# chaoting-sun/GCT-Plus

Hardware: AMD Instinct MI355X
Metric: SMILES/sec training step (vaetf, seq_len=80, d_model=512) (higher is better)
Workload: dtype f32

## Files before the change

gct_plus_amd/csrc/attention.hip:

```cpp
#include "common.h"

typedef float f32x4 __attribute__((ext_vector_type(4)));

namespace {

constexpr int ATT_THREADS = 384;
constexpr int MASK_W = 8;
constexpr int L_MAX = 208;
constexpr int DIRECT_NT = GCT_ATTN_DIRECT_MAX_KEYS / 16;
constexpr int mask_words(int nt) { return (nt + 1) / 2; }
static_assert(GCT_ATTN_DIRECT_MAX_KEYS % 32 == 0 && mask_words(DIRECT_NT) == GCT_ATTN_DIRECT_MAX_KEYS / 32,
              "the direct kernels' rows are whole mask words");

struct AttnArgs {
  const float *q, *k, *v;
  int ldq, ldk, ldv;
  const uint32_t* mbits;
  int mb_sb, mb_sq;
  const uint32_t* tbits;
  int tb_sb, tb_su;
  float* o;
  int ldo;
  float* lse;
  float* probs;
  const float *o_in, *dout, *lse_in;
  float *dq, *dk, *dv;
  int lddq, lddk, lddv;
  const int32_t *cstart, *nlive;
  int kv_compact;
  int qo_compact;
  const int32_t *kstart, *klen;
  float4* ws_meta;
  uint32_t* ws_keep;
  uint32_t* ws_use;
  int B, H, Lq, Lk, npairs;
  float scale, keep_scale;
  uint32_t thr;
  GctRng rng;
#ifdef GCT_STAMPS
  unsigned long long* stamps;
#endif
};

#ifdef GCT_STAMPS
#define ASTAMP_DECL unsigned long long seg[8] = {0, 0, 0, 0, 0, 0, 0, 0}, tprev; \
  asm volatile("s_memtime %0\n\ts_waitcnt lgkmcnt(0)" : "=s"(tprev)::"memory")
#define ASTAMP(i)                                                                      \
  do {                                                                                 \
    __builtin_amdgcn_sched_barrier(0);                                                 \
    unsigned long long t__;                                                            \
    asm volatile("s_memtime %0\n\ts_waitcnt lgkmcnt(0)" : "=s"(t__)::"memory");         \
    __builtin_amdgcn_sched_barrier(0);                                                 \
    seg[i] += t__ - tprev;                                                             \
    tprev = t__;                                                                       \
  } while (0)
#define GCT_STAMP_ITEM0 8192
#define DSTAMP_OUT_AT(item, rec0)                                                      \
  if (a.stamps && (threadIdx.x & 63) == 0 && (item) >= GCT_STAMP_ITEM0 && (item) < GCT_STAMP_ITEM0 + 4096)  \
    for (int i = 0; i < 8; ++i) a.stamps[((size_t)((item) - GCT_STAMP_ITEM0 + (rec0))) * 8 + i] = seg[i]
#define DSTAMP_OUT(item) DSTAMP_OUT_AT(item, 0)
#else
#define ASTAMP_DECL
#define ASTAMP(i)
#define DSTAMP_OUT(item)
#define DSTAMP_OUT_AT(item, rec0)
#endif

__device__ __forceinline__ f32x4 mfma16(float a, float b, f32x4 c) {
  return __builtin_amdgcn_mfma_f32_16x16x4f32(a, b, c, 0, 0, 0);
}

template <int DK, int NT>
struct StageOff {
  static constexpr int C = DK / 4;
  static constexpr int ITERS = (16 * NT * C + ATT_THREADS - 1) / ATT_THREADS;
  uint32_t off[ITERS];
  __device__ __forceinline__ void init(int ld, int L, int tid) {
#pragma unroll
    for (int it = 0; it < ITERS; ++it) {
      const int idx = tid + it * ATT_THREADS;
      const int r = idx / C, c = idx - r * C;
      off[it] = (uint32_t)(((r < L ? r : L - 1) * ld + c * 4) * 4);
    }
  }
};
template <int DK, int NT>
struct Stage {
  static constexpr int SD = DK + 4, C = DK / 4;
  static constexpr int ITERS = StageOff<DK, NT>::ITERS;
  float4 v[ITERS];
  __device__ __forceinline__ void load(const float* src, int ld, int b, int h, int L, const StageOff<DK, NT>& o) {
    const float* base = src + (int64_t)b * L * ld + h * DK;
#pragma unroll
    for (int it = 0; it < ITERS; ++it)
      v[it] = *reinterpret_cast<const float4*>(reinterpret_cast<const char*>(base) + o.off[it]);
  }
  __device__ __forceinline__ void load_rows(const float* src, int ld, int64_t row0, int h, const StageOff<DK, NT>& o) {
    const float* base = src + row0 * ld + h * DK;
#pragma unroll
    for (int it = 0; it < ITERS; ++it)
      v[it] = *reinterpret_cast<const float4*>(reinterpret_cast<const char*>(base) + o.off[it]);
  }
  __device__ __forceinline__ void store(float* dst, int L, int LP, int tid) const {
#pragma unroll
    for (int it = 0; it < ITERS; ++it) {
      const int idx = tid + it * ATT_THREADS;
      const int r = idx / C, c = idx - r * C;
      if (r < LP)
        *reinterpret_cast<float4*>(dst + r * SD + c * 4) = r < L ? v[it] : make_float4(0.f, 0.f, 0.f, 0.f);
    }
  }
};

template <int NDT>
// ... 211 lines not shown
    sv.load_rows(a.v, a.ldv, kr0, h, kvo);
    row_frag_global<NDT>(bq, a.q, a.ldq, b, h, a.Lq, 16 * wave + c16, g);
    if (a.mbits) mask_row_raw<MW>(mraw, a, b, 16 * wave + c16);
  }
  for (;;) {
    const int b = pair / a.H, h = pair - b * a.H;
    const int Lk_in = a.klen ? a.klen[b] : a.Lk;
    sk.store(Ks, Lk_in, LKP, tid);
    sv.store(Vs, Lk_in, LKP, tid);
    uint32_t mw[MW];
    mask_row_use<MW>(mw, mraw, a, 16 * wave + c16);
    __syncthreads();
    const int next = pair + (int)gridDim.x;
    const bool more = next < a.npairs;
    const int nb = more ? next / a.H : b, nh = more ? next - nb * a.H : h;
    const int64_t nkr0 = a.kstart ? (int64_t)a.kstart[nb] : (int64_t)nb * a.Lk;
    if (PIPE && more) {
      sk.load_rows(a.k, a.ldk, nkr0, nh, kvo);
      sv.load_rows(a.v, a.ldv, nkr0, nh, kvo);
      if (a.mbits) mask_row_raw<MW>(mraw, a, nb, 16 * wave + c16);
    }
    for (int u = wave; u < nqt; u += NW) {
      if (u != wave) {
        row_frag_global<NDT>(bq, a.q, a.ldq, b, h, a.Lq, 16 * u + c16, g);
        uint4 r2[(MW + 3) / 4] = {};
        if (a.mbits) mask_row_raw<MW>(r2, a, b, 16 * u + c16);
        mask_row_use<MW>(mw, r2, a, 16 * u + c16);
      }
      const bool last = u + NW >= nqt;
      fwd_unit<NDT, NT, true>(a, b, h, u, bq, mw, Ks, Vs, nkt, lane, [&]() {
        if (PIPE && more && last) row_frag_global<NDT>(bq, a.q, a.ldq, nb, nh, a.Lq, 16 * wave + c16, g);
      });
    }
    if (PIPE && more && wave >= nqt) row_frag_global<NDT>(bq, a.q, a.ldq, nb, nh, a.Lq, 16 * wave + c16, g);
    if (!more) break;
    __syncthreads();
    if (!PIPE) {
      sk.load_rows(a.k, a.ldk, nkr0, nh, kvo);
      sv.load_rows(a.v, a.ldv, nkr0, nh, kvo);
      row_frag_global<NDT>(bq, a.q, a.ldq, nb, nh, a.Lq, 16 * wave + c16, g);
      if (a.mbits) mask_row_raw<MW>(mraw, a, nb, 16 * wave + c16);
    }
    pair = next;
  }
}

typedef float f32x2 __attribute__((ext_vector_type(2)));
template <int NDT> struct VecN;
template <> struct VecN<4> { typedef f32x4 T; };
template <> struct VecN<2> { typedef f32x2 T; };
template <> struct VecN<1> { typedef float T; };
template <int NDT> __device__ __forceinline__ float vec_at(const typename VecN<NDT>::T& v, int i);
template <> __device__ __forceinline__ float vec_at<4>(const f32x4& v, int i) { return v[i]; }
template <> __device__ __forceinline__ float vec_at<2>(const f32x2& v, int i) { return v[i]; }
template <> __device__ __forceinline__ float vec_at<1>(const float& v, int) { return v; }

template <int NDT>
struct WaveTile {
  static constexpr int SD = 16 * NDT + 4;
  typedef typename VecN<NDT>::T VT;
  float* t;
  __device__ __forceinline__ void put(const VT (&v)[4], int g, int c16) const {
#pragma unroll
    for (int r = 0; r < 4; ++r) *reinterpret_cast<VT*>(t + (4 * g + r) * SD + NDT * c16) = v[r];
  }
  __device__ __forceinline__ void get(float4 (&f)[NDT], int g, int c16) const {
    __builtin_amdgcn_wave_barrier();
#pragma unroll
    for (int j = 0; j < NDT; ++j) f[j] = *reinterpret_cast<const float4*>(t + c16 * SD + g * 4 * NDT + 4 * j);
    __builtin_amdgcn_wave_barrier();
  }
};
template <int NDT>
__device__ __forceinline__ void tile_load(typename VecN<NDT>::T (&v)[4], const char* base, int ld, int row0, int last,
                                          int g, int c16) {
  typedef typename VecN<NDT>::T VT;
#pragma unroll
  for (int r = 0; r < 4; ++r) {
    const int rr = row0 + 4 * g + r;
    v[r] = *reinterpret_cast<const VT*>(base + (uint32_t)(((rr < last ? rr : last) * ld + NDT * c16) * 4));
  }
}

template <int NDT, int NT>
__global__ __launch_bounds__(256, 6) void attn_fwd_direct_kernel(const AttnArgs a) {
  constexpr int DK = 16 * NDT, MW = mask_words(NT);
  typedef typename VecN<NDT>::T VT;
  const int lane = threadIdx.x & 63, g = lane >> 4, c16 = lane & 15;
  const int nqt = (a.Lq + 15) >> 4, nkt = (a.Lk + 15) >> 4;
  const int item = __builtin_amdgcn_readfirstlane((int)blockIdx.x * 4 + (int)(threadIdx.x >> 6));
  if (item >= a.npairs * nqt) return;
  ASTAMP_DECL;
  const int pair = item / nqt, u = item - pair * nqt;
  const int b = pair / a.H, h = pair - b * a.H;
  const int q = 16 * u + c16;
  const int Lq_e = a.qo_compact ? a.nlive[b] : a.Lq;
  const int64_t qr0 = a.qo_compact ? (int64_t)a.cstart[b] : (int64_t)b * a.Lq;
  if (16 * u >= Lq_e) return;
  const int Lk_in = a.klen ? a.klen[b] : a.Lk;
  const int64_t kr0 = a.kstart ? (int64_t)a.kstart[b] : (int64_t)b * a.Lk;
  const int klast = Lk_in > 0 ? Lk_in - 1 : 0;
  __shared__ __attribute__((aligned(16))) float tiles[4][16 * WaveTile<NDT>::SD];
  const int wv = threadIdx.x >> 6;
  const WaveTile<NDT> T0{tiles[wv]}, T1{tiles[wv]};
  VT tq[4];
  tile_load<NDT>(tq, reinterpret_cast<const char*>(a.q + qr0 * a.ldq + h * DK), a.ldq, 16 * u, Lq_e - 1, g, c16);
  uint4 mraw[(MW + 3) / 4] = {};
  if (a.mbits) mask_row_raw<MW>(mraw, a, b, q);
  const char* kbase = reinterpret_cast<const char*>(a.k + kr0 * a.ldk + h * DK);
  VT tk[4];
  uint32_t use = 0;
  if (a.tbits) {
    use = __builtin_amdgcn_readfirstlane(a.tbits[(int64_t)b * a.tb_sb + u * a.tb_su]);
    if (use & 1u) tile_load<NDT>(tk, kbase, a.ldk, 0, klast, g, c16);
  }
  uint32_t mw[MW];
  mask_row_use<MW>(mw, mraw, a, q);
  if (!a.tbits) {
    use = tiles_for_q<MW>(mw, q, a.Lq, a.Lk, nkt);
    if (use & 1u) tile_load<NDT>(tk, kbase, a.ldk, 0, klast, g, c16);
  }
  ASTAMP(0);
  uint32_t rowvis = 0;
#pragma unroll
  for (int w = 0; w < MW; ++w) rowvis |= mw[w] & range_word(w, a.Lk);
  float4 bq[NDT];
  T1.put(tq, g, c16);
  T1.get(bq, g, c16);
  ASTAMP(1);
  f32x4 sacc[NT];
#pragma unroll
  for (int t = 0; t < NT; ++t) sacc[t] = (f32x4){0.f, 0.f, 0.f, 0.f};
#pragma unroll
  for (int t = 0; t < NT; ++t) {
    if (t > 0 && ((use >> t) & 1u))
      tile_load<NDT>(tk, kbase, a.ldk, 16 * t, klast, g, c16);
    if ((use >> t) & 1u) {
      float4 ak[NDT];
      if (t & 1) {
        T1.put(tk, g, c16);
        T1.get(ak, g, c16);
      } else {
        T0.put(tk, g, c16);
        T0.get(ak, g, c16);
      }
      sacc[t] = dot_frag<NDT>(ak, bq, sacc[t]);
    }
  }
  ASTAMP(2);
  const char* vbase = reinterpret_cast<const char*>(a.v + kr0 * a.ldv + h * DK);
  VT av[4];
  if (use & 1u) tile_load<NDT>(av, vbase, a.ldv, 0, klast, g, c16);
  ASTAMP(3);
  float m = -INFINITY;
#pragma unroll
  for (int t = 0; t < NT; ++t)
    if ((use >> t) & 1u) {
      const uint32_t nib = mw[t >> 1] >> ((t & 1) * 16 + 4 * g);
#pragma unroll
      for (int r = 0; r < 4; ++r) {
        const float sv = score_of(sacc[t][r] * a.scale, 16 * t + 4 * g + r < a.Lk, (nib >> r) & 1u);
        sacc[t][r] = sv;
        m = fmaxf(m, sv);
      }
    }
  m = fmaxf(m, __shfl_xor(m, 16, 64));
  m = fmaxf(m, __shfl_xor(m, 32, 64));
  if (m == -INFINITY) m = 0.f;
  float l = 0.f;
#pragma unroll
  for (int t = 0; t < NT; ++t)
    if ((use >> t) & 1u) {
#pragma unroll
      for (int r = 0; r < 4; ++r) {
        const float e = __expf(sacc[t][r] - m);
        sacc[t][r] = e;
        l += e;
      }
    }
  l += __shfl_xor(l, 16, 64);
// ... 261 lines not shown
      const int kw = k >> 5, kb = k & 31;
      const bool inr = k < a.Lk;
#pragma unroll 1
      for (int u = 0; u < nqt; ++u) {
        if (!__any(rowlive[16 * u + c16] != 0)) continue;
        uint32_t vis4 = 0;
#pragma unroll
        for (int r = 0; r < 4; ++r) vis4 |= ((mb_s[(16 * u + 4 * g + r) * MW + kw] >> kb) & 1u) << r;
        const bool ok = __all(rowok[16 * u + c16] != 0);
        if (ok && !__any(inr && vis4 != 0)) continue;
        uint32_t keep4 = 0xfu;
        if (a.thr) {
          keep4 = 0;
#pragma unroll
          for (int r = 0; r < 4; ++r) keep4 |= ((kp_s[(16 * u + 4 * g + r) * MW + kw] >> kb) & 1u) << r;
        }
        f32x4 sa = (f32x4){0.f, 0.f, 0.f, 0.f}, pa = (f32x4){0.f, 0.f, 0.f, 0.f};
        {
          float4 aq[NDT], ad[NDT];
          row_frag<NDT>(aq, R0, 16 * u + c16, g);
          row_frag<NDT>(ad, R1, 16 * u + c16, g);
          sa = dot_frag<NDT>(aq, bk, sa);
          pa = dot_frag<NDT>(ad, bv, pa);
        }
        float pd[4], ds[4];
#pragma unroll
        for (int r = 0; r < 4; ++r) {
          const int qq = 16 * u + 4 * g + r;
          const bool vis = (vis4 >> r) & 1u, keep = (keep4 >> r) & 1u;
          const float p = inr ? __expf(score_of(sa[r] * a.scale, true, vis, rowok[qq] ? -1e9f : 0.f) - lse_s[qq]) : 0.f;
          const float dpd = keep ? pa[r] * a.keep_scale : 0.f;
          pd[r] = keep ? p * a.keep_scale : 0.f;
          ds[r] = (inr && vis) ? p * (dpd - del_s[qq]) : 0.f;
        }
#pragma unroll
        for (int r = 0; r < 4; ++r) {
          const float* dorow = R1 + (16 * u + 4 * g + r) * SD + c16;
          const float* qrow = R0 + (16 * u + 4 * g + r) * SD + c16;
#pragma unroll
          for (int dt = 0; dt < NDT; ++dt) {
            vacc[dt] = mfma16(dorow[16 * dt], pd[r], vacc[dt]);
            kacc[dt] = mfma16(qrow[16 * dt], ds[r], kacc[dt]);
          }
        }
      }
      if (k < Lk_e) {
        char* vbase = reinterpret_cast<char*>(a.dv + krow0 * a.lddv + h * DK);
        char* kbase = reinterpret_cast<char*>(a.dk + krow0 * a.lddk + h * DK);
        const uint32_t voff = (uint32_t)((k * a.lddv + 4 * g) * 4), koff = (uint32_t)((k * a.lddk + 4 * g) * 4);
#pragma unroll
        for (int dt = 0; dt < NDT; ++dt) {
          *reinterpret_cast<float4*>(vbase + voff + 64 * dt) = make_float4(vacc[dt][0], vacc[dt][1], vacc[dt][2], vacc[dt][3]);
          *reinterpret_cast<float4*>(kbase + koff + 64 * dt) =
              make_float4(kacc[dt][0] * a.scale, kacc[dt][1] * a.scale, kacc[dt][2] * a.scale, kacc[dt][3] * a.scale);
        }
      }
    }
    __syncthreads();
  }
}

template <int NDT>
struct DqBuf {
  typename VecN<NDT>::T kt[4], vt[4];
};

template <int NDT, int NT>
__global__ __launch_bounds__(256, 4) void attn_bwd_dq_kernel(const AttnArgs a) {
  constexpr int DK = 16 * NDT, MW = mask_words(NT);
  const int lane = threadIdx.x & 63, g = lane >> 4, c16 = lane & 15;
  const int nqt = (a.Lq + 15) >> 4, nkt = (a.Lk + 15) >> 4, LQP = 16 * nqt;
  const int item = __builtin_amdgcn_readfirstlane((int)blockIdx.x * 4 + (int)(threadIdx.x >> 6));
  if (item >= a.npairs * nqt) return;
  ASTAMP_DECL;
  const int pair = item / nqt, u = item - pair * nqt;
  const int b = pair / a.H, h = pair - b * a.H;
  const int64_t lrow0 = (int64_t)pair * a.Lq;
  const int Lq_e = a.nlive ? a.nlive[b] : a.Lq;
  const int64_t drow0 = a.cstart ? (int64_t)a.cstart[b] : (int64_t)b * a.Lq;
  const int64_t kin0 = a.kstart ? (int64_t)a.kstart[b] : (int64_t)b * a.Lk;
  const int Lk_in = a.klen ? a.klen[b] : a.Lk;
  const int klast = Lk_in > 0 ? Lk_in - 1 : 0;
  uint32_t* visit = a.ws_use + (int64_t)pair * nqt + u;
  if (16 * u >= Lq_e) {
    if (lane == 0) *visit = 0;
    return;
  }
  const int q = 16 * u + c16;
  const bool real = q < Lq_e;
  __shared__ __attribute__((aligned(16))) float tiles[4][2][16 * WaveTile<NDT>::SD];
  const int wv = threadIdx.x >> 6;
  const WaveTile<NDT> T0{tiles[wv][0]}, T1{tiles[wv][1]};
  DqBuf<NDT> b0;
  float4 bq[NDT], bd[NDT];
  float del = 0.f;
  int nz = 0;
  float lse0;
  uint4 mraw[(MW + 3) / 4] = {};
  {
    float4 bo[NDT];
    const int64_t qrow0 = a.qo_compact ? drow0 : (int64_t)b * a.Lq;
    const int qlast = (a.qo_compact ? Lq_e : a.Lq) - 1;
    const char* qb = reinterpret_cast<const char*>(a.q + qrow0 * a.ldq + h * DK);
    const char* db = reinterpret_cast<const char*>(a.dout + drow0 * a.ldo + h * DK);
    const char* ob = reinterpret_cast<const char*>(a.o_in + qrow0 * a.ldo + h * DK);
    tile_load<NDT>(b0.kt, qb, a.ldq, 16 * u, qlast, g, c16);
    tile_load<NDT>(b0.vt, db, a.ldo, 16 * u, Lq_e - 1, g, c16);
    lse0 = a.lse_in[lrow0 + (q < a.Lq ? q : a.Lq - 1)];
    if (a.mbits) mask_row_raw<MW>(mraw, a, b, q);
    T0.put(b0.kt, g, c16);
    T0.get(bq, g, c16);
    T1.put(b0.vt, g, c16);
    tile_load<NDT>(b0.kt, ob, a.ldo, 16 * u, qlast, g, c16);
    T1.get(bd, g, c16);
    T0.put(b0.kt, g, c16);
    T0.get(bo, g, c16);
#pragma unroll
    for (int j = 0; j < NDT; ++j) {
      del += (bo[j].x * bd[j].x + bo[j].y * bd[j].y) + (bo[j].z * bd[j].z + bo[j].w * bd[j].w);
      nz |= (bd[j].x != 0.f) | (bd[j].y != 0.f) | (bd[j].z != 0.f) | (bd[j].w != 0.f);
    }
  }
  ASTAMP(0);
  del += __shfl_xor(del, 16, 64);
  del += __shfl_xor(del, 32, 64);
  nz |= __shfl_xor(nz, 16, 64);
  nz |= __shfl_xor(nz, 32, 64);
  del = real ? del : 0.f;
  nz = real ? nz : 0;
  const float lse = real ? lse0 : 0.f;
  uint32_t mw[MW];
  mask_row_use<MW>(mw, mraw, a, q);
  uint32_t rowvis = 0;
#pragma unroll
  for (int w = 0; w < MW; ++w) rowvis |= mw[w] & range_word(w, a.Lk);
  const float masked = rowvis ? -1e9f : 0.f;
  if (g == 0) a.ws_meta[(int64_t)pair * LQP + q] = make_float4(lse, del, masked, nz ? 1.f : 0.f);
  const bool tile_live = __any(nz);
  char* dbase = reinterpret_cast<char*>(a.dq + drow0 * a.lddq + h * DK);
  const uint32_t doff = (uint32_t)((q * a.lddq + 4 * NDT * g) * 4);
  if (!tile_live) {
    if (lane == 0) *visit = 0;
    if (real) {
#pragma unroll
      for (int i = 0; i < NDT; ++i) *reinterpret_cast<float4*>(dbase + doff + 16 * i) = make_float4(0.f, 0.f, 0.f, 0.f);
    }
    return;
  }
  const uint32_t use = a.tbits ? __builtin_amdgcn_readfirstlane(a.tbits[(int64_t)b * a.tb_sb + u * a.tb_su])
                               : tiles_for_q<MW>(mw, q, a.Lq, a.Lk, nkt);
  if (lane == 0) *visit = use;
  const uint64_t keepw = keep_bits_row<NT>(a, (uint32_t)(lrow0 + q), use, g);
  ASTAMP(1);
  uint16_t* kp_h = reinterpret_cast<uint16_t*>(a.ws_keep + ((int64_t)pair * LQP + q) * MW);
  const char* kbase = reinterpret_cast<const char*>(a.k + kin0 * a.ldk + h * DK);
  const char* vbase = reinterpret_cast<const char*>(a.v + kin0 * a.ldv + h * DK);
  auto load = [&](DqBuf<NDT>& B_, int t) {
    tile_load<NDT>(B_.kt, kbase, a.ldk, 16 * t, klast, g, c16);
    tile_load<NDT>(B_.vt, vbase, a.ldv, 16 * t, klast, g, c16);
  };
  f32x4 qacc[NDT];
#pragma unroll
  for (int dt = 0; dt < NDT; ++dt) qacc[dt] = (f32x4){0.f, 0.f, 0.f, 0.f};
  auto compute = [&](const DqBuf<NDT>& B_, int t) {
    ASTAMP(2);
    f32x4 sacc = (f32x4){0.f, 0.f, 0.f, 0.f}, pacc = (f32x4){0.f, 0.f, 0.f, 0.f};
    {
      float4 ak[NDT];
      T0.put(B_.kt, g, c16);
      T0.get(ak, g, c16);
      sacc = dot_frag<NDT>(ak, bq, sacc);
      T1.put(B_.vt, g, c16);
      T1.get(ak, g, c16);
      pacc = dot_frag<NDT>(ak, bd, pacc);
    }
    ASTAMP(3);
    uint32_t word = mw[0];
#pragma unroll
    for (int w = 1; w < MW; ++w) word = (t >> 1) == w ? mw[w] : word;
    const uint32_t nib = word >> ((t & 1) * 16 + 4 * g);
    const uint32_t keep = (uint32_t)(keepw >> (4 * t)) & 0xfu;
    if (a.thr) {
      uint32_t hw = keep << (4 * g);
      hw |= __shfl_xor(hw, 16, 64);
      hw |= __shfl_xor(hw, 32, 64);
      if (g == 0) kp_h[t] = (uint16_t)hw;
    }
    float ds[4];
#pragma unroll
    for (int r = 0; r < 4; ++r) {
      const bool inr = 16 * t + 4 * g + r < a.Lk, vis = (nib >> r) & 1u;
      const float p = inr ? __expf(score_of(sacc[r] * a.scale, true, vis, masked) - lse) : 0.f;
      const float dpd = ((keep >> r) & 1u) ? pacc[r] * a.keep_scale : 0.f;
      ds[r] = (inr && vis) ? p * (dpd - del) : 0.f;
    }
    ASTAMP(4);
#pragma unroll
    for (int r = 0; r < 4; ++r) {
#pragma unroll
      for (int dt = 0; dt < NDT; ++dt) qacc[dt] = mfma16(vec_at<NDT>(B_.kt[r], dt), ds[r], qacc[dt]);
    }
    ASTAMP(5);
  };
  for (uint32_t rem = use; rem; rem &= rem - 1) {
    const int t0 = __builtin_ctz(rem);
    load(b0, t0);
    compute(b0, t0);
  }
  if (real) {
#pragma unroll
    for (int i = 0; i < 4; ++i) {
      if constexpr (NDT == 4)
        *reinterpret_cast<float4*>(dbase + doff + 16 * i) =
            make_float4(qacc[0][i] * a.scale, qacc[1][i] * a.scale, qacc[2][i] * a.scale, qacc[3][i] * a.scale);
      else if constexpr (NDT == 2)
        *reinterpret_cast<float2*>(dbase + doff + 8 * i) = make_float2(qacc[0][i] * a.scale, qacc[1][i] * a.scale);
      else
        *reinterpret_cast<float*>(dbase + doff + 4 * i) = qacc[0][i] * a.scale;
    }
  }
  ASTAMP(6);
  DSTAMP_OUT_AT(item, 4096);
}

template <int NDT>
struct DkvBuf {
  typename VecN<NDT>::T tq[4], td[4];
};

template <int NDT, int NT>
__global__ __launch_bounds__(256, 4) void attn_bwd_dkv_kernel(const AttnArgs a) {
  constexpr int DK = 16 * NDT, MW = mask_words(NT);
  const int lane = threadIdx.x & 63, g = lane >> 4, c16 = lane & 15;
  const int nqt = (a.Lq + 15) >> 4, nkt = (a.Lk + 15) >> 4, LQP = 16 * nqt;
  const int item = __builtin_amdgcn_readfirstlane((int)blockIdx.x * 4 + (int)(threadIdx.x >> 6));
  if (item >= a.npairs * nkt) return;
  ASTAMP_DECL;
  const int pair = item / nkt, t = item - pair * nkt;
  const int b = pair / a.H, h = pair - b * a.H;
  const int Lq_e = a.nlive ? a.nlive[b] : a.Lq;
  const int64_t drow0 = a.cstart ? (int64_t)a.cstart[b] : (int64_t)b * a.Lq;
  const int64_t kin0 = a.kstart ? (int64_t)a.kstart[b] : (int64_t)b * a.Lk;
  const int Lk_in = a.klen ? a.klen[b] : a.Lk;
  const int Lk_e = a.kv_compact ? Lq_e : Lk_in;
  const int64_t krow0 = a.kv_compact ? drow0 : kin0;
  if (16 * t >= Lk_e) return;
  const int k = 16 * t + c16;
  const bool inr = k < a.Lk;
  uint32_t rem = 0;
  {
    const uint32_t* vw = a.ws_use + (int64_t)pair * nqt;
    const int Lq_x = Lq_e < a.Lq ? Lq_e : a.Lq;
    const int nqt_e = (Lq_x + 15) >> 4;
    for (int u = 0; u < nqt_e; ++u) rem |= ((vw[u] >> t) & 1u) << u;
    rem = __builtin_amdgcn_readfirstlane(rem);
  }
  __shared__ __attribute__((aligned(16))) float tiles[4][2][16 * WaveTile<NDT>::SD];
  const int wv = threadIdx.x >> 6;
  const WaveTile<NDT> T0{tiles[wv][0]}, T1{tiles[wv][1]};
  float4 bk[NDT], bv[NDT];
  DkvBuf<NDT> b0;
  {
    DkvBuf<NDT>& kv = b0;
    const char* kb0 = reinterpret_cast<const char*>(a.k + kin0 * a.ldk + h * DK);
    const char* vb0 = reinterpret_cast<const char*>(a.v + kin0 * a.ldv + h * DK);
    const int klast = Lk_in > 0 ? Lk_in - 1 : 0;
    tile_load<NDT>(kv.tq, kb0, a.ldk, 16 * t, klast, g, c16);
    tile_load<NDT>(kv.td, vb0, a.ldv, 16 * t, klast, g, c16);
    T0.put(kv.tq, g, c16);
    T1.put(kv.td, g, c16);
    T0.get(bk, g, c16);
    T1.get(bv, g, c16);
  }
  ASTAMP(0);
  f32x4 vacc[NDT], kacc[NDT];
#pragma unroll
  for (int dt = 0; dt < NDT; ++dt) {
    vacc[dt] = (f32x4){0.f, 0.f, 0.f, 0.f};
    kacc[dt] = (f32x4){0.f, 0.f, 0.f, 0.f};
  }
  const int kw = t >> 1, kb = (t & 1) * 16 + c16;
  const float4* meta = a.ws_meta + (int64_t)pair * LQP;
  const uint32_t* kp = a.ws_keep + (int64_t)pair * LQP * MW + kw;
  const uint32_t* mb = a.mbits ? a.mbits + (int64_t)b * a.mb_sb + kw : nullptr;
  const int64_t qrow0 = a.qo_compact ? drow0 : (int64_t)b * a.Lq;
  const int qlast = (a.qo_compact ? Lq_e : a.Lq) - 1;
  const char* qbase = reinterpret_cast<const char*>(a.q + qrow0 * a.ldq + h * DK);
  const char* dbase = reinterpret_cast<const char*>(a.dout + drow0 * a.ldo + h * DK);
  auto load = [&](DkvBuf<NDT>& B_, int u) {
    tile_load<NDT>(B_.tq, qbase, a.ldq, 16 * u, qlast, g, c16);
    tile_load<NDT>(B_.td, dbase, a.ldo, 16 * u, Lq_e - 1, g, c16);
  };
  auto compute = [&](const DkvBuf<NDT>& B_, int u) {
    float4 mt[4];
    uint32_t mword[4], kword[4];
    {
      const int qq = 16 * u + 4 * g + (c16 & 3);
      const int qc = qq < a.Lq ? qq : a.Lq - 1;
      const float4 m1 = meta[qq];
      const uint32_t w1 = mb ? mb[qc * a.mb_sq] : 0xffffffffu;
      const uint32_t k1 = a.thr ? kp[qq * MW] : 0xffffffffu;
#define GCT_QUAD(v, r) __builtin_amdgcn_mov_dpp((int)(v), (r) * 0x55, 0xf, 0xf, true)
#pragma unroll
      for (int r = 0; r < 4; ++r) {
        mt[r].x = __int_as_float(r == 0 ? GCT_QUAD(__float_as_int(m1.x), 0) : r == 1 ? GCT_QUAD(__float_as_int(m1.x), 1)
                               : r == 2 ? GCT_QUAD(__float_as_int(m1.x), 2) : GCT_QUAD(__float_as_int(m1.x), 3));
        mt[r].y = __int_as_float(r == 0 ? GCT_QUAD(__float_as_int(m1.y), 0) : r == 1 ? GCT_QUAD(__float_as_int(m1.y), 1)
                               : r == 2 ? GCT_QUAD(__float_as_int(m1.y), 2) : GCT_QUAD(__float_as_int(m1.y), 3));
        mt[r].z = __int_as_float(r == 0 ? GCT_QUAD(__float_as_int(m1.z), 0) : r == 1 ? GCT_QUAD(__float_as_int(m1.z), 1)
                               : r == 2 ? GCT_QUAD(__float_as_int(m1.z), 2) : GCT_QUAD(__float_as_int(m1.z), 3));
        mt[r].w = 0.f;
        mword[r] = (uint32_t)(r == 0 ? GCT_QUAD(w1, 0) : r == 1 ? GCT_QUAD(w1, 1) : r == 2 ? GCT_QUAD(w1, 2) : GCT_QUAD(w1, 3));
        kword[r] = (uint32_t)(r == 0 ? GCT_QUAD(k1, 0) : r == 1 ? GCT_QUAD(k1, 1) : r == 2 ? GCT_QUAD(k1, 2) : GCT_QUAD(k1, 3));
      }
#undef GCT_QUAD
    }
    ASTAMP(1);
    f32x4 sa = (f32x4){0.f, 0.f, 0.f, 0.f}, pa = (f32x4){0.f, 0.f, 0.f, 0.f};
    {
      float4 aq[NDT];
      T0.put(B_.tq, g, c16);
      T1.put(B_.td, g, c16);
      T0.get(aq, g, c16);
      sa = dot_frag<NDT>(aq, bk, sa);
      T1.get(aq, g, c16);
      pa = dot_frag<NDT>(aq, bv, pa);
    }
    ASTAMP(2);
// ... 193 lines not shown
  const int per_cu = lds <= 50 * 1024 ? 3 : lds <= 76 * 1024 ? 2 : 1;
  const int64_t want = (int64_t)cus * per_cu * 2;
  return {nt8 ? AttnRoute::LDS8 : AttnRoute::LDS13, npairs < want ? npairs : want, 0, lds};
}

struct BwdWs {
  int64_t keep, use, bytes;
};
BwdWs bwd_ws_layout(int B, int H, int Lq) {
  const int64_t LQP = (Lq + 15) & ~15, rows = (int64_t)B * H * LQP;
  const int64_t keep = rows * 16, use = keep + rows * mask_words(DIRECT_NT) * 4;
  return {keep, use, use + (((int64_t)B * H * (LQP / 16) * 4 + 15) & ~(int64_t)15)};
}

template <typename K>
int launch_lds(K kernel, const AttnRoute& r, const AttnArgs& a, hipStream_t st) {
  int rc = ensure_lds(kernel, r.lds);
  if (rc) return rc;
  hipLaunchKernelGGL(kernel, dim3((unsigned)r.grid), dim3(ATT_THREADS), r.lds, st, a);
  return GCT_OK;
}

template <bool BWD, int NDT>
int launch_route(const AttnRoute& r, const AttnArgs& a, hipStream_t st) {
  switch (r.kind) {
    case AttnRoute::DIRECT:
      if constexpr (BWD) {
        hipLaunchKernelGGL((attn_bwd_dq_kernel<NDT, DIRECT_NT>), dim3((unsigned)r.grid), dim3(256), 0, st, a);
        hipLaunchKernelGGL((attn_bwd_dkv_kernel<NDT, DIRECT_NT>), dim3((unsigned)r.grid_kv), dim3(256), 0, st, a);
      } else {
        hipLaunchKernelGGL((attn_fwd_direct_kernel<NDT, DIRECT_NT>), dim3((unsigned)r.grid), dim3(256), 0, st, a);
      }
      return GCT_OK;
    case AttnRoute::LDS8:
      return BWD ? launch_lds(attn_bwd_kernel<NDT, 8>, r, a, st) : launch_lds(attn_fwd_kernel<NDT, 8>, r, a, st);
    default:
      return BWD ? launch_lds(attn_bwd_kernel<NDT, 13>, r, a, st) : launch_lds(attn_fwd_kernel<NDT, 13>, r, a, st);
  }
}

template <bool BWD>
int launch(int dk, const AttnRoute& r, const AttnArgs& a, hipStream_t st) {
  switch (dk) {
    case 64: return launch_route<BWD, 4>(r, a, st);
    case 32: return launch_route<BWD, 2>(r, a, st);
    default: return launch_route<BWD, 1>(r, a, st);
  }
}

}

extern "C" int gct_attn_mask_pack(const uint8_t* mask, int64_t mask_sb, int64_t mask_sq, int B, int Lq, int Lk,
                                  uint32_t* bits, uint32_t* tiles, void* stream) {
  GCT_CHECK_ARG(mask && bits && B >= 0 && Lq > 0 && Lk > 0 && Lk <= 32 * MASK_W && gct_aligned16(bits),
                "attn_mask_pack: bad args (Lk <= %d)", 32 * MASK_W);
  const int rows = mask_sq == 0 ? 1 : Lq;
  const int64_t n = (int64_t)B * rows * MASK_W;
  if (n == 0) return GCT_OK;
  hipLaunchKernelGGL(mask_pack_kernel, dim3((unsigned)((n + 255) / 256)), dim3(256), 0, (hipStream_t)stream, mask,
                     mask_sb, mask_sq, B, rows, Lk, bits);
  GCT_LAUNCH_CHECK("attn_mask_pack");
  if (tiles) {
    const int ntr = mask_sq == 0 ? 1 : (Lq + 15) / 16;
    const int64_t items = (int64_t)B * ntr;
    hipLaunchKernelGGL(mask_tiles_kernel, dim3((unsigned)((items + 3) / 4)), dim3(256), 0, (hipStream_t)stream, bits,
                       rows * MASK_W, mask_sq == 0 ? 0 : MASK_W, B, ntr, Lq, Lk, tiles);
    GCT_LAUNCH_CHECK("attn_mask_pack (tiles)");
  }
  return GCT_OK;
}

extern "C" int gct_trg_mask_tokens(const int64_t* tokens, int64_t ld_tok, int64_t pad, int B, int T, uint8_t* out,
                                   void* stream) {
  GCT_CHECK_ARG(tokens && out && B >= 0 && T > 0 && ld_tok >= T && ((uintptr_t)out & 3u) == 0,
                "trg_mask_tokens: bad args");
  const int64_t n4 = ((int64_t)B * T * T + 3) / 4;
  if (n4 == 0) return GCT_OK;
  hipLaunchKernelGGL(trg_mask_tokens_kernel, dim3((unsigned)((n4 + 255) / 256)), dim3(256), 0, (hipStream_t)stream,
                     tokens, ld_tok, pad, B, T, out);
  GCT_LAUNCH_CHECK("trg_mask_tokens");
  return GCT_OK;
}

extern "C" int gct_attn_fwd(const float* q, int64_t ldq, const float* k, int64_t ldk,
                            const float* v, int64_t ldv, const uint32_t* mbits, int64_t mb_sb,
                            int64_t mb_sq, float* o, int64_t ldo, float* lse, float* probs, int B,
                            int H, int Lq, int Lk, int dk, float scale, float p, uint64_t seed,
                            uint32_t site, const int32_t* kstart, const int32_t* klen, const uint32_t* tbits,
                            int64_t tb_sb, int64_t tb_su, const int32_t* qstart, const int32_t* qlen, void* stream) {
  int rc = check_common("attn_fwd", q, ldq, k, ldk, v, ldv, mbits, mb_sb, mb_sq, B, H, Lq, Lk, dk, p);
  if (rc) return rc;
  GCT_CHECK_ARG(o && lse && ldo % 4 == 0 && gct_aligned16(o) && (int64_t)Lq * ldo * 4 < (1ll << 31), "attn_fwd: bad output");
  if (B == 0) return GCT_OK;
  AttnArgs a = {};
  a.q = q; a.k = k; a.v = v; a.ldq = (int)ldq; a.ldk = (int)ldk; a.ldv = (int)ldv;
  a.mbits = mbits; a.mb_sb = (int)mb_sb; a.mb_sq = (int)mb_sq;
  a.o = o; a.ldo = (int)ldo; a.lse = lse; a.probs = probs;
  a.tbits = tbits; a.tb_sb = (int)tb_sb; a.tb_su = (int)tb_su;
#ifdef GCT_STAMPS
  a.stamps = g_attn_stamps;
#endif
  GCT_CHECK_ARG((kstart == nullptr) == (klen == nullptr), "attn_fwd: kstart / klen go together");
  a.kstart = kstart; a.klen = klen;
  GCT_CHECK_ARG((qstart == nullptr) == (qlen == nullptr), "attn_fwd: qstart / qlen go together");
  GCT_CHECK_ARG(!qstart || (Lk <= GCT_ATTN_DIRECT_MAX_KEYS && !probs),
                "attn_fwd: compact query rows need the direct kernel (Lk <= %d) and no probs output",
                GCT_ATTN_DIRECT_MAX_KEYS);
  a.cstart = qstart; a.nlive = qlen; a.qo_compact = qstart ? 1 : 0;
  a.B = B; a.H = H; a.Lq = Lq; a.Lk = Lk; a.npairs = B * H; a.scale = scale;
  a.thr = gct_drop_threshold(p); a.keep_scale = 1.0f / (1.0f - p); a.rng = gct_rng_make(seed, site);
  rc = launch<false>(dk, plan_attn_fwd(Lq, Lk, dk, a.npairs, num_cus()), a, (hipStream_t)stream);
  if (rc) return rc;
  GCT_LAUNCH_CHECK("attn_fwd");
  return GCT_OK;
}

extern "C" int64_t gct_attn_bwd_ws_bytes(int B, int H, int Lq, int Lk) {
  if (B <= 0 || H <= 0 || Lq <= 0 || Lk <= 0 || Lk > GCT_ATTN_DIRECT_MAX_KEYS) return 0;
  return bwd_ws_layout(B, H, Lq).bytes;
}

extern "C" int gct_attn_bwd(const float* q, int64_t ldq, const float* k, int64_t ldk,
                            const float* v, int64_t ldv, const uint32_t* mbits, int64_t mb_sb,
                            int64_t mb_sq, const float* o, const float* dout, int64_t ldo,
                            const float* lse, float* dq, int64_t lddq, float* dk_,
                            int64_t lddk, float* dv, int64_t lddv, int B, int H, int Lq, int Lk,
                            int dk, float scale, float p, uint64_t seed, uint32_t site,
                            const int32_t* cstart, const int32_t* nlive, int kv_compact,
                            const int32_t* kstart, const int32_t* klen, const uint32_t* tbits, int64_t tb_sb,
                            int64_t tb_su, void* ws, int64_t ws_bytes, void* stream) {
  int rc = check_common("attn_bwd", q, ldq, k, ldk, v, ldv, mbits, mb_sb, mb_sq, B, H, Lq, Lk, dk, p);
  if (rc) return rc;
  GCT_CHECK_ARG(o && dout && lse && dq && dk_ && dv, "attn_bwd: null pointer");
  GCT_CHECK_ARG(ldo % 4 == 0 && lddq % 4 == 0 && lddk % 4 == 0 && lddv % 4 == 0 &&
                    gct_aligned16(o) && gct_aligned16(dout) && gct_aligned16(dq) &&
                    gct_aligned16(dk_) && gct_aligned16(dv),
                "attn_bwd: buffers must be 16-B aligned with ld %% 4 == 0");
  GCT_CHECK_ARG((int64_t)Lq * (ldo > lddq ? ldo : lddq) * 4 < (1ll << 31) && (int64_t)Lk * (lddk > lddv ? lddk : lddv) * 4 < (1ll << 31),
                "attn_bwd: one (batch) slice exceeds 2 GiB");
  if (B == 0) return GCT_OK;
  AttnArgs a = {};
  a.q = q; a.k = k; a.v = v; a.ldq = (int)ldq; a.ldk = (int)ldk; a.ldv = (int)ldv;
  a.mbits = mbits; a.mb_sb = (int)mb_sb; a.mb_sq = (int)mb_sq;
  a.o_in = o; a.dout = dout; a.ldo = (int)ldo; a.lse_in = lse;
  a.tbits = tbits; a.tb_sb = (int)tb_sb; a.tb_su = (int)tb_su;
  a.dq = dq; a.dk = dk_; a.dv = dv; a.lddq = (int)lddq; a.lddk = (int)lddk; a.lddv = (int)lddv;
#ifdef GCT_STAMPS
  a.stamps = g_attn_stamps;
#endif
  const int qo_compact = (kv_compact >> 1) & 1;
  kv_compact &= 1;
  GCT_CHECK_ARG((cstart == nullptr) == (nlive == nullptr) && (!kv_compact || (cstart && Lq == Lk)),
                "attn_bwd: cstart / nlive go together; kv_compact needs them and Lq == Lk");
  GCT_CHECK_ARG(!qo_compact || cstart, "attn_bwd: compact q / o rows need cstart / nlive");
  a.cstart = cstart; a.nlive = nlive; a.kv_compact = kv_compact; a.qo_compact = qo_compact;
  GCT_CHECK_ARG((kstart == nullptr) == (klen == nullptr) && !(kstart && kv_compact),
                "attn_bwd: kstart / klen go together and exclude kv_compact");
  a.kstart = kstart; a.klen = klen;
  GCT_CHECK_ARG(!qo_compact || Lk <= GCT_ATTN_DIRECT_MAX_KEYS,
                "attn_bwd: compact q / o rows need the direct kernels (Lk <= %d)", GCT_ATTN_DIRECT_MAX_KEYS);
  const int64_t ws_need = gct_attn_bwd_ws_bytes(B, H, Lq, Lk);
  GCT_CHECK_ARG(ws_need == 0 || (ws && gct_aligned16(ws) && ws_bytes >= ws_need),
                "attn_bwd: Lk <= %d needs a 16-B aligned workspace of %lld B (gct_attn_bwd_ws_bytes); got %lld B at %p",
                GCT_ATTN_DIRECT_MAX_KEYS, (long long)ws_need, (long long)ws_bytes, ws);
  a.B = B; a.H = H; a.Lq = Lq; a.Lk = Lk; a.npairs = B * H; a.scale = scale;
  a.thr = gct_drop_threshold(p); a.keep_scale = 1.0f / (1.0f - p); a.rng = gct_rng_make(seed, site);
  const AttnRoute r = plan_attn_bwd(Lq, Lk, dk, a.npairs, num_cus());
  GCT_CHECK_ARG(r.grid <= INT32_MAX && r.grid_kv <= INT32_MAX, "attn_bwd: grid too large");
  if (r.kind == AttnRoute::DIRECT) {
    const BwdWs w = bwd_ws_layout(B, H, Lq);
    a.ws_meta = reinterpret_cast<float4*>(ws);
    a.ws_keep = reinterpret_cast<uint32_t*>(static_cast<char*>(ws) + w.keep);
    a.ws_use = reinterpret_cast<uint32_t*>(static_cast<char*>(ws) + w.use);
  }
  rc = launch<true>(dk, r, a, (hipStream_t)stream);
  if (rc) return rc;
  GCT_LAUNCH_CHECK("attn_bwd");
  return GCT_OK;
}
```

gct_plus_amd/csrc/gemm.hip:

```cpp
#include <limits.h>
#include <stdlib.h>

#include "common.h"

typedef float f32x16 __attribute__((ext_vector_type(16)));

namespace {

constexpr int BM = 128, BN = 128, BK = 32;
constexpr int TILE_FLOATS = BM * BK;

struct Seg3 {
  const float* p0;
  int64_t d1, d2;
};

struct GemmArgs {
  int64_t M, N, K;
  Seg3 a;
  int64_t lda;
  int64_t a_nper;
  Seg3 b;
  int64_t ldb;
  int64_t b_nper;
// ... 240 lines not shown
#ifdef GCT_STAMPS
  unsigned long long seg[8] = {0, 0, 0, 0, 0, 0, 0, 0}, tprev;
  asm volatile("s_memtime %0\n\ts_waitcnt lgkmcnt(0)" : "=s"(tprev)::"memory");
#endif
  if (nkt > 0) {
    gload(kbeg);
    lstore(0);
  }
  __syncthreads();
  STAMP(0);
  for (int64_t kt = 0; kt < nkt; ++kt) {
    const int cur = (int)(kt & 1);
    if (kt + 1 < nkt) gload(kbeg + (kt + 1) * BK);
    STAMP(1);
    const float* la = lds + cur * 2 * TILE_FLOATS;
    const float* lb = la + TILE_FLOATS;
    float fa[2][2][4], fb[2][2][4];
    auto fragq = [&](int set, int c) {
      if (A_KC) fragq_kc(fa[set], la, wm, lane, c); else fragq_rc(fa[set], la, wm, lane, c);
      if (B_KC) fragq_kc(fb[set], lb, wn, lane, c); else fragq_rc(fb[set], lb, wn, lane, c);
    };
    fragq(0, 0);
#pragma unroll
    for (int c = 0; c < 4; ++c) {
      const int set = c & 1;
      if (c < 3) fragq(set ^ 1, c + 1);
      __builtin_amdgcn_sched_barrier(0);
#pragma unroll
      for (int e = 0; e < 4; ++e) {
#pragma unroll
        for (int i = 0; i < 2; ++i)
#pragma unroll
          for (int j = 0; j < 2; ++j)
            acc[i][j] = __builtin_amdgcn_mfma_f32_32x32x2f32(fa[set][i][e], fb[set][j][e], acc[i][j],
                                                             0, 0, 0);
      }
      __builtin_amdgcn_sched_barrier(0);
    }
    STAMP(2);
#ifdef GCT_STAMPS
    asm volatile("s_waitcnt vmcnt(0)" ::: "memory");
    STAMP(3);
#endif
    if (kt + 1 < nkt) lstore(cur ^ 1);
    STAMP(4);
    __syncthreads();
    STAMP(5);
  }

  const int h = lane >> 5;
#pragma unroll
  for (int i = 0; i < 2; ++i) {
#pragma unroll
    for (int j = 0; j < 2; ++j) {
      const int64_t col = n0 + wn + j * 32 + (lane & 31);
      if (col >= g.N) continue;
      int64_t cloc;
      float* cbase;
      float bias = 0.f;
      if (g.epi == EPI_SLAB) {
        cbase = g.c0 + (int64_t)z * g.slab_stride;
        cloc = col;
      } else {
        const bool g1 = col >= g.c_nper, g2 = col >= 2 * g.c_nper;
        cloc = col - (g2 ? 2 * g.c_nper : (g1 ? g.c_nper : 0));
        cbase = g.c0 + (g2 ? g.c_d2 : (g1 ? g.c_d1 : 0));
        if (g.epi < EPI_D0 && g.bias0)
          bias = g.bias0[(g2 ? g.bias_d2 : (g1 ? g.bias_d1 : 0)) + cloc];
      }
#pragma unroll
      for (int q4 = 0; q4 < 4; ++q4) {
        const int64_t row_base = m0 + wm + i * 32 + 8 * q4 + 4 * h;
        uint4 bits = make_uint4(~0u, ~0u, ~0u, ~0u);
        const bool need_rng = g.thr != 0u && (g.epi == GCT_EPI_GELU_DROP ||
                                              g.epi == GCT_EPI_GELU_DROP_SAVE ||
                                              g.epi == GCT_EPI_DROP_RESID ||
                                              g.epi == EPI_D0 + GCT_DEPI_GELU_BWD);
        if (need_rng) bits = gct_drop_bits(g.rng, drop_quad(g, row_base), (uint32_t)col);
#pragma unroll
        for (int e = 0; e < 4; ++e) {
          const int64_t row = row_base + e;
          if (row >= g.M) continue;
          float v = acc[i][j][q4 * 4 + e];
          const int64_t off = row * g.ldc + cloc;
          const bool keep = gct_drop_keep(bits, e, (uint32_t)col, g.thr);
          switch (g.epi) {
            case GCT_EPI_BIAS:
              v += bias;
              break;
            case GCT_EPI_GELU_DROP: {
              v += bias;
              g.pre[off] = v;
              v = gct_gelu(v);
              v = keep ? v * g.keep_scale : 0.f;
            } break;
            case GCT_EPI_GELU_DROP_SAVE: {
              float gd;
              const float y = gct_gelu_with_grad(v + bias, gd);
              g.pre[off] = keep ? gd : 0.f;
              v = keep ? y * g.keep_scale : 0.f;
            } break;
            case GCT_EPI_DROP_RESID: {
              v += bias;
              v = keep ? v * g.keep_scale : 0.f;
              v += g.resid[off];
            } break;
            case EPI_D0 + GCT_DEPI_ACCUM:
              v += cbase[off];
              break;
            case EPI_D0 + GCT_DEPI_GELU_BWD: {
              float u = 0.f;
              if (g.pre_rows > 0) {
                const int64_t er0 = pre_row0(g, row_base);
                if (er0 >= 0 && er0 + e < g.pre_rows) u = g.pre_in[(er0 + e) * g.ldc + cloc];
              } else {
                u = g.pre_in[off];
              }
              v = keep ? v * gct_gelu_grad(u) * g.keep_scale : 0.f;
            } break;
            case EPI_D0 + GCT_DEPI_MUL_SAVED: {
              float d = 0.f;
              if (g.pre_rows > 0) {
                const int64_t er0 = pre_row0(g, row_base);
                if (er0 >= 0 && er0 + e < g.pre_rows) d = g.pre_in[(er0 + e) * g.ldc + cloc];
              } else {
                d = g.pre_in[off];
              }
              v = d == 0.f ? 0.f : v * d * g.keep_scale;
            } break;
            default:
              break;
          }
          cbase[off] = v;
        }
      }
    }
  }
#ifdef GCT_STAMPS
  STAMP(6);
  if (g.stamps && (threadIdx.x & 63) == 0 && blockIdx.x < 64) {
    for (int i = 0; i < 8; ++i) g.stamps[((size_t)blockIdx.x * 4 + (threadIdx.x >> 6)) * 8 + i] = seg[i];
  }
#endif
}


typedef float f32x4_t __attribute__((ext_vector_type(4)));
__device__ __forceinline__ void epi_store4(float* p, const float (&x)[4]) {
#ifdef GCT_LAB_NO_EPI_STORE
  if (x[0] != 123456.789f) return;
#endif
  __builtin_nontemporal_store(f32x4_t{x[0], x[1], x[2], x[3]}, reinterpret_cast<f32x4_t*>(p));
}

template <int SIDE>
struct FastEpiT {
  static constexpr bool FWD = SIDE == 0 || SIDE == 1, BWD = SIDE == 0 || SIDE == 2;
  const GemmArgs& g;
  __device__ __forceinline__ bool needs_extra() const {
#ifdef GCT_LAB_NO_EPI_MATH
    return false;
#endif
    return (FWD && g.epi == GCT_EPI_DROP_RESID) || (BWD && g.epi == EPI_D0 + GCT_DEPI_ACCUM) || reads_pre();
  }
  __device__ __forceinline__ bool reads_pre() const {
    return BWD && (g.epi == EPI_D0 + GCT_DEPI_GELU_BWD || g.epi == EPI_D0 + GCT_DEPI_MUL_SAVED);
  }
  __device__ __forceinline__ const float* extra_base(const float* cbase) const {
    return (FWD && g.epi == GCT_EPI_DROP_RESID) ? g.resid : (reads_pre() ? g.pre_in : cbase);
  }
  __device__ __forceinline__ void prefetch(float4 (&x)[4], int64_t row0, const float* cbase,
                                           int64_t cloc) const {
    const float* eb = extra_base(cbase);
    int64_t er0 = row0, elim = g.M;
    if (reads_pre() && g.pre_rows > 0) {
      er0 = pre_row0(g, row0);
      elim = er0 < 0 ? -1 : g.pre_rows;
    }
#pragma unroll
    for (int rr = 0; rr < 4; ++rr) {
      x[rr] = make_float4(0.f, 0.f, 0.f, 0.f);
      if (row0 + rr < g.M && er0 + rr < elim) x[rr] = *reinterpret_cast<const float4*>(eb + (er0 + rr) * g.ldc + cloc);
    }
  }
  __device__ __forceinline__ void apply(float4 (&v)[4], int64_t row0, int64_t col0,
                                        float* cbase, int64_t cloc, float4 bias) const {
    float4 x[4];
    if (needs_extra()) prefetch(x, row0, cbase, cloc);
    apply(v, x, row0, col0, cbase, cloc, bias);
  }
  __device__ __forceinline__ void apply(float4 (&v)[4], const float4 (&ex)[4], int64_t row0,
                                        int64_t col0, float* cbase, int64_t cloc, float4 bias) const {
#ifdef GCT_LAB_NO_EPI_MATH
    const int epi = EPI_D0 + GCT_DEPI_STORE;
#else
    const int epi = g.epi;
#endif
    uint4 bits[2];
    const bool rng = g.thr != 0u && ((FWD && (epi == GCT_EPI_GELU_DROP || epi == GCT_EPI_GELU_DROP_SAVE ||
                                              epi == GCT_EPI_DROP_RESID)) ||
                                     (BWD && epi == EPI_D0 + GCT_DEPI_GELU_BWD));
    if (rng) {
#pragma unroll
      for (int cp = 0; cp < 2; ++cp)
        bits[cp] = gct_drop_bits(g.rng, drop_quad(g, row0), (uint32_t)(col0 + 2 * cp));
    }
#pragma unroll
    for (int rr = 0; rr < 4; ++rr) {
      const int64_t row = row0 + rr;
      if (row >= g.M) break;
      const int64_t off = row * g.ldc + cloc;
      float x[4] = {v[rr].x, v[rr].y, v[rr].z, v[rr].w};
      const float bs[4] = {bias.x, bias.y, bias.z, bias.w};
      bool keep[4] = {true, true, true, true};
      if (rng) {
#pragma unroll
        for (int cc = 0; cc < 4; ++cc) keep[cc] = gct_drop_keep(bits[cc >> 1], rr, (uint32_t)cc, g.thr);
      }
      if (FWD && epi == GCT_EPI_BIAS) {
#pragma unroll
        for (int cc = 0; cc < 4; ++cc) x[cc] += bs[cc];
      } else if (FWD && epi == GCT_EPI_GELU_DROP) {
#pragma unroll
        for (int cc = 0; cc < 4; ++cc) x[cc] += bs[cc];
        epi_store4(g.pre + off, x);
#pragma unroll
        for (int cc = 0; cc < 4; ++cc) x[cc] = keep[cc] ? gct_gelu(x[cc]) * g.keep_scale : 0.f;
      } else if (FWD && epi == GCT_EPI_GELU_DROP_SAVE) {
        float d[4];
#pragma unroll
        for (int cc = 0; cc < 4; ++cc) {
          float gd;
          const float y = gct_gelu_with_grad(x[cc] + bs[cc], gd);
          d[cc] = keep[cc] ? gd : 0.f;
          x[cc] = keep[cc] ? y * g.keep_scale : 0.f;
        }
        epi_store4(g.pre + off, d);
      } else if (FWD && epi == GCT_EPI_DROP_RESID) {
        const float4 r = ex[rr];
        const float rs[4] = {r.x, r.y, r.z, r.w};
#pragma unroll
        for (int cc = 0; cc < 4; ++cc)
          x[cc] = (keep[cc] ? (x[cc] + bs[cc]) * g.keep_scale : 0.f) + rs[cc];
      } else if (BWD && epi == EPI_D0 + GCT_DEPI_ACCUM) {
        const float4 r = ex[rr];
        x[0] += r.x; x[1] += r.y; x[2] += r.z; x[3] += r.w;
      } else if (BWD && epi == EPI_D0 + GCT_DEPI_GELU_BWD) {
        const float4 u = ex[rr];
        const float us[4] = {u.x, u.y, u.z, u.w};
#pragma unroll
        for (int cc = 0; cc < 4; ++cc)
          x[cc] = keep[cc] ? x[cc] * gct_gelu_grad(us[cc]) * g.keep_scale : 0.f;
      } else if (BWD && epi == EPI_D0 + GCT_DEPI_MUL_SAVED) {
        const float4 u = ex[rr];
        const float ds[4] = {u.x, u.y, u.z, u.w};
#pragma unroll
        for (int cc = 0; cc < 4; ++cc) x[cc] = ds[cc] == 0.f ? 0.f : x[cc] * ds[cc] * g.keep_scale;
      }
      epi_store4(cbase + off, x);
    }
  }
};
using FastEpi = FastEpiT<0>;


template <int SIDE>
__device__ __forceinline__ void wave_epilogue_tail(const GemmArgs& g, float* stg, int lane, int64_t mw,
                                                   int64_t nw, unsigned z);
template <int SIDE>
__device__ __forceinline__ void wave_epilogue(const GemmArgs& g, const f32x16 (&acc)[2][2], float* stg,
                                              int lane, int64_t mw, int64_t nw, unsigned z) {
  {
    const int h = lane >> 5, c32 = lane & 31;
#pragma unroll
    for (int i = 0; i < 2; ++i)
#pragma unroll
      for (int j = 0; j < 2; ++j)
#pragma unroll
        for (int r = 0; r < 16; ++r)
          stg[(i * 32 + (r & 3) + 8 * (r >> 2) + 4 * h) * 64 + j * 32 + c32] = acc[i][j][r];
  }
  wave_epilogue_tail<SIDE>(g, stg, lane, mw, nw, z);
}

template <int SIDE>
__device__ __forceinline__ void wave_epilogue_tail(const GemmArgs& g, float* stg, int lane, int64_t mw,
                                                   int64_t nw, unsigned z) {
  __builtin_amdgcn_s_waitcnt(0xC07F);
  __builtin_amdgcn_wave_barrier();
  const FastEpiT<SIDE> ep{g};
  const int c4 = lane & 15;
  const int64_t col0 = nw + c4 * 4;
  if (col0 < g.N) {
    float* cbase;
    int64_t cloc;
    float4 bias = make_float4(0.f, 0.f, 0.f, 0.f);
    if (g.epi == EPI_SLAB) {
      cbase = g.c0 + (int64_t)z * g.slab_stride;
      cloc = col0;
    } else {
      const bool g1 = col0 >= g.c_nper, g2 = col0 >= 2 * g.c_nper;
      cloc = col0 - (g2 ? 2 * g.c_nper : (g1 ? g.c_nper : 0));
      cbase = g.c0 + (g2 ? g.c_d2 : (g1 ? g.c_d1 : 0));
      if (g.epi < EPI_D0 && g.bias0)
        bias = *reinterpret_cast<const float4*>(g.bias0 + (g2 ? g.bias_d2 : (g1 ? g.bias_d1 : 0)) + cloc);
    }
    float4 ex[4][4];
    const bool extra = ep.needs_extra();
    if (extra) {
#pragma unroll
      for (int it = 0; it < 4; ++it)
        ep.prefetch(ex[it], mw + (it * 4 + (lane >> 4)) * 4, cbase, cloc);
    }
#pragma unroll
    for (int it = 0; it < 4; ++it) {
      const int rg = it * 4 + (lane >> 4);
      const int64_t row0 = mw + rg * 4;
      if (row0 >= g.M) continue;
      float4 v[4];
#pragma unroll
      for (int rr = 0; rr < 4; ++rr)
        v[rr] = *reinterpret_cast<const float4*>(stg + (rg * 4 + rr) * 64 + c4 * 4);
      ep.apply(v, ex[it], row0, col0, cbase, cloc, bias);
    }
  }
}

// ... 502 lines not shown
  if (tiles <= 0) return 1;
  int64_t ns = 768 / tiles;
  if (ns > K / BK / 4) ns = K / BK / 4;
  return ns < 1 ? 1 : (int)ns;
}

int x6_tail_plan(int64_t M, int64_t N, int64_t K, int64_t* m1_out) {
  constexpr int64_t CUS = 256;
  const int64_t tm = (M + XBM - 1) / XBM, tn = (N + XBN - 1) / XBN, tiles = tm * tn;
  const int64_t rem = tiles % CUS;
  if (tiles <= CUS || rem == 0 || rem % tn != 0 || K % XBK != 0) return 1;
  const int64_t nkt = K / XBK;
  int best = 1;
  double cost = 1.0;
  const double o = 3.3;
  for (int s2 = 2; s2 <= 8 && nkt / s2 >= 2; ++s2) {
    const double c = (double)((rem * s2 + CUS - 1) / CUS) * (o + (double)nkt / s2) / (o + nkt) + 0.05;
    if (c < cost - 1e-9) { cost = c; best = s2; }
  }
  if (best == 1 || cost > 0.75) return 1;
  *m1_out = (tiles - rem) / tn * XBM;
  return best;
}

int x6_splitk_all_plan(int64_t M, int64_t N, int64_t K) {
  constexpr int64_t CUS = 256;
  const int64_t tiles = ((M + XBM - 1) / XBM) * ((N + XBN - 1) / XBN), nkt = K / XBK;
  if (tiles > CUS / 2 || K % XBK != 0 || nkt < 32 || M < 1024 || (nkt < 64 && M < 2048)) return 1;
  int64_t sp = CUS / tiles;
  if (sp > nkt / 8) sp = nkt / 8;
  if (sp > 8) sp = 8;
  return sp < 2 ? 1 : (int)sp;
}


inline int64_t x6s_tiles(int64_t M, int64_t N) { return ((M + SBM - 1) / SBM) * ((N + SBN - 1) / SBN); }

inline bool x6s_shape(const GemmArgs& g) {
  const int64_t big = ((g.M + XBM - 1) / XBM) * ((g.N + XBN - 1) / XBN), small = x6s_tiles(g.M, g.N), nkt = g.K / XBK;
  return big <= 160 && small >= 96 && small <= (nkt <= 16 ? 512 : 256) && nkt <= 32;
}

constexpr int64_t X6_TAIL_SMALL_MAX = 512;

constexpr int64_t PANEL32_MAX_TILES = 4096, PANEL64_MAX_TILES = 768;


static_assert(BK == XBK, "the fp32 and bf16x6 kernels split K at the same granularity");
GemmArgs slab_args(const GemmArgs& g, int splits, float* ws) {
  const int64_t nkt = g.K / BK;
  GemmArgs p = g;
  p.ksplit = ((nkt + splits - 1) / splits) * BK;
  p.nsplit = (int)((g.K + p.ksplit - 1) / p.ksplit);
  p.epi = EPI_SLAB; p.c0 = ws; p.ldc = g.N; p.slab_stride = g.M * g.N;
  p.c_d1 = p.c_d2 = 0; p.c_nper = INT64_MAX / 4; p.bias0 = nullptr; p.resid = nullptr; p.pre = nullptr; p.pre_in = nullptr;
  return p;
}

int launch_fixup(const GemmArgs& g, const GemmArgs& slabs, hipStream_t st, const char* name) {
  const int64_t patches = ((g.M + 3) / 4) * (g.N / 4);
  hipLaunchKernelGGL(splitk_epilogue_kernel, dim3((unsigned)((patches + 255) / 256)), dim3(256), 0, st, g,
                     (const float*)slabs.c0, slabs.nsplit, slabs.slab_stride);
  GCT_LAUNCH_CHECK(name);
  return GCT_OK;
}

template <int MODE, int NP>
int launch_x6_tail_split(const GemmArgs& g, hipStream_t st, float* ws, int64_t ws_bytes) {
  if (MODE == X6_WGRAD || g.nsplit != 1 || !ws || !gct_aligned16(ws)) return launch_x6<MODE, NP>(g, st);
  int64_t m1 = 0;
  const int best = x6_tail_plan(g.M, g.N, g.K, &m1);
  const int64_t m2 = g.M - m1, nkt = g.K / XBK;
  hipStreamCaptureStatus cap = hipStreamCaptureStatusNone;
  if (best == 1 || slab_bytes(best, m2, g.N) > ws_bytes ||
      hipStreamIsCapturing(st, &cap) != hipSuccess || cap != hipStreamCaptureStatusNone)
    return launch_x6<MODE, NP>(g, st);
  GemmArgs head = g;
  head.M = m1;
  int rc = launch_x6<MODE, NP>(head, st);
  if (rc) return rc;
  GemmArgs e = g;
  e.M = m2; e.row_base = g.row_base + m1;
  e.a.p0 += m1 * g.lda;
  e.c0 += m1 * g.ldc;
  if (e.resid) e.resid += m1 * g.ldc;
  if (e.pre) e.pre += m1 * g.ldc;
  if (e.pre_in && !(g.pre_rows > 0 && g.quad_map)) e.pre_in += m1 * g.ldc;
  if (nkt <= 32 && x6s_tiles(m2, g.N) <= X6_TAIL_SMALL_MAX) {
    if (MODE == X6_FWD && x6s_ok(e, true)) return launch_x6s<X6_FWD, NP>(e, st);
    if (MODE == X6_DGRAD && x6s_dgrad_ok(e, true)) return launch_x6s<X6_DGRAD, NP>(e, st);
  }
  const GemmArgs p = slab_args(e, best, ws);
  rc = launch_x6<MODE, NP>(p, st);
  if (rc) return rc;
  return launch_fixup(e, p, st, "x6 tail fix-up");
}

struct GemmRoute {
  enum Kind {
    X6S,
    X6_SPLITK_ALL,
    PANEL_THIN,
    PANEL32,
    PANEL64,
    F32_SMALL,
    X6,
    F32_FAST,
    F32_VEC,
    F32,
  } kind;
  int splits;
};

template <bool A_KC, bool B_KC>
GemmRoute plan_gemm(const GemmArgs& g, bool vec, int mode, const float* ws, int64_t ws_bytes) {
  constexpr bool FWD = A_KC && B_KC, DGRAD = A_KC && !B_KC;
  constexpr int MODE = A_KC ? (B_KC ? X6_FWD : X6_DGRAD) : X6_WGRAD;
  const bool x6 = mode == GCT_GEMM_BF16X6 || mode == GCT_GEMM_BF16X3;
  const bool x6_fwd = x6 && FWD && g.epi < EPI_D0, x6_dgrad = x6 && DGRAD && g.epi >= EPI_D0 && g.epi < EPI_SLAB;
  const bool ws_ok = ws && gct_aligned16(ws);
  if (x6_fwd || x6_dgrad) {
    const bool x6s = x6_fwd ? x6s_ok(g, vec) : x6s_dgrad_ok(g, vec);
    if (x6s && x6s_shape(g)) return {GemmRoute::X6S, 1};
    if (x6_fwd && x6s && !x6_ok<X6_FWD>(g, vec) && x6s_tiles(g.M, g.N) >= 96) return {GemmRoute::X6S, 1};
    const int sp = x6_splitk_all_plan(g.M, g.N, g.K);
    if (x6_ok<MODE>(g, vec) && g.nsplit == 1 && ws_ok && sp > 1 && slab_bytes(sp, g.M, g.N) <= ws_bytes)
      return {GemmRoute::X6_SPLITK_ALL, sp};
  }
  if (FWD && vec && g.N <= 32 && g.K % 256 == 0 && g.epi == GCT_EPI_BIAS && g.nsplit == 1 && g.b_nper >= g.N &&
      g.c_nper >= g.N && g.M >= 1 && g.lda * 4 * 33 < (1ll << 31) && g.ldb * 4 * 33 < (1ll << 31) && g.M < (1ll << 36))
    return {GemmRoute::PANEL_THIN, 1};
  const bool fast = fast_ok<A_KC, B_KC>(g, vec);
  if (FWD && fast && g.nsplit == 1 && skinny_m(g.M, g.N) && g.epi < EPI_D0 && (g.b_nper >= g.N || g.b_nper % 64 == 0)) {
    if (g.K % 256 == 0 && g.lda * 4 * 33 < (1ll << 31) && g.ldb * 4 * 65 < (1ll << 31) &&
        (g.c_nper >= g.N || g.c_nper % 64 == 0)) {
      const int64_t tm32 = (g.M + 31) / 32;
      if (g.N % 32 == 0 && (g.b_nper >= g.N || g.b_nper % 32 == 0) && tm32 * (g.N / 32) <= PANEL32_MAX_TILES)
        return {GemmRoute::PANEL32, 1};
      if (g.N % 64 == 0 && tm32 * (g.N / 64) <= PANEL64_MAX_TILES) return {GemmRoute::PANEL64, 1};
    }
    int64_t ns = 1;
    if (ws_ok) {
      const int64_t slab = g.M * g.N * (int64_t)sizeof(float);
      ns = skinny_splits(g.M, g.N, g.K);
      if (ns * slab > ws_bytes) ns = ws_bytes / slab;
      if (ns < 1) ns = 1;
    }
    return {GemmRoute::F32_SMALL, (int)ns};
  }
  if (x6 && (A_KC || !B_KC) && x6_ok<MODE>(g, vec)) return {GemmRoute::X6, 1};
  return {fast ? GemmRoute::F32_FAST : (vec ? GemmRoute::F32_VEC : GemmRoute::F32), 1};
}

template <bool A_KC, bool B_KC>
int launch(const GemmArgs& g, bool vec, hipStream_t st, float* ws = nullptr, int64_t ws_bytes = 0) {
  constexpr int MODE = A_KC ? (B_KC ? X6_FWD : X6_DGRAD) : X6_WGRAD;
  const int64_t tiles = ((g.M + BM - 1) / BM) * ((g.N + BN - 1) / BN) * g.nsplit;
  if (tiles <= 0) return GCT_OK;
  if (tiles > INT_MAX) {
    gct_set_error("gemm: grid too large");
    return GCT_ERR_ARG;
  }
  const int mode = gemm_mode();
  const bool x3 = mode == GCT_GEMM_BF16X3;
  const GemmRoute r = plan_gemm<A_KC, B_KC>(g, vec, mode, ws, ws_bytes);
  switch (r.kind) {
    case GemmRoute::X6S:
// ... 103 lines not shown
  GCT_CHECK_ARG(epi >= GCT_EPI_BIAS && epi <= GCT_EPI_GELU_DROP_SAVE, "linear_fwd: unknown epilogue %d", epi);
  GCT_CHECK_ARG((epi != GCT_EPI_GELU_DROP && epi != GCT_EPI_GELU_DROP_SAVE) || pre, "linear_fwd: GELU epilogue needs pre");
  GCT_CHECK_ARG(epi != GCT_EPI_DROP_RESID || resid, "linear_fwd: residual epilogue needs resid");
  GCT_CHECK_ARG(p >= 0.f && p < 1.f, "linear_fwd: dropout p out of range");
  GemmArgs g = {};
  g.M = M; g.N = (int64_t)nseg * nper; g.K = K;
  GCT_CHECK_ARG(!b0 || nseg < 2 || b1, "linear_fwd: bias of segment 1 missing");
  GCT_CHECK_ARG(!b0 || nseg < 3 || b2, "linear_fwd: bias of segment 2 missing");
  g.a = mkseg(x, nullptr, nullptr); g.lda = ldx; g.a_nper = INT64_MAX / 4;
  g.b = mkseg(w0, w1, w2); g.ldb = ldw; g.b_nper = nper;
  g.c0 = y0; g.c_d1 = y1 ? y1 - y0 : 0; g.c_d2 = y2 ? y2 - y0 : 0; g.ldc = ldy; g.c_nper = nper;
  g.ksplit = K; g.nsplit = 1; g.epi = epi;
  g.bias0 = b0; g.bias_d1 = (b0 && b1) ? b1 - b0 : 0; g.bias_d2 = (b0 && b2) ? b2 - b0 : 0;
  g.resid = resid; g.pre = pre;
  g.thr = gct_drop_threshold(p); g.keep_scale = 1.0f / (1.0f - p); g.rng = gct_rng_make(seed, site);
  g.bp0 = wp0; g.bp_stride = plane_stride;
  g.quad_map = quad_map;
  const bool vec = al16(x) && al16(w0) && al16(w1) && al16(w2) && (ldx % 4 == 0) &&
                   (ldw % 4 == 0) && (K % 4 == 0);
  return launch<true, true>(g, vec, (hipStream_t)stream, ws, ws ? ws_bytes : 0);
}

extern "C" int gct_gemm_set_mode(int mode) {
  GCT_CHECK_ARG(mode == GCT_GEMM_F32 || mode == GCT_GEMM_BF16X6 || mode == GCT_GEMM_BF16X3,
                "gemm_set_mode: unknown mode %d", mode);
  g_gemm_mode = mode;
  return GCT_OK;
}
extern "C" int gct_gemm_get_mode(void) { return gemm_mode(); }
extern "C" int64_t gct_gemm_x6_kernel_launches(void) { return g_x6_kernel_launches; }
extern "C" int64_t gct_gemm_x3_launches(void) { return g_x3_kernel_launches; }
extern "C" int gct_gemm_launch_counts(int64_t* out2) {
  GCT_CHECK_ARG(out2, "gemm_launch_counts: null");
  out2[0] = g_gemm_launches[0]; out2[1] = g_gemm_launches[1];
  return GCT_OK;
}

extern "C" int gct_split_planes(const float* src, int64_t numel, uint16_t* planes, int64_t plane_stride,
                                void* stream) {
  GCT_CHECK_ARG(src && planes && numel >= 0 && numel % 4 == 0 && plane_stride >= numel && plane_stride % 4 == 0 &&
                    gct_aligned16(src) && ((((uintptr_t)planes) & 7u) == 0),
                "split_planes: bad args (numel and plane_stride must be multiples of 4, src 16-B aligned)");
  if (numel == 0) return GCT_OK;
  const int64_t n4 = numel / 4;
  hipLaunchKernelGGL(split_planes_kernel, dim3((unsigned)((n4 + 255) / 256)), dim3(256), 0, (hipStream_t)stream,
                     src, planes, n4, plane_stride);
  GCT_LAUNCH_CHECK("split_planes");
  return GCT_OK;
}

extern "C" int64_t gct_linear_fwd_ws_bytes(int64_t M, int K, int Ntot) {
  int64_t need = 0, m1 = 0;
  if (skinny_m(M, Ntot)) {
    need = slab_bytes(skinny_splits(M, Ntot, K), M, Ntot);
  } else {
    const int s = x6_tail_plan(M, Ntot, K, &m1);
    need = slab_bytes(s, M - m1, Ntot);
  }
  const int64_t all = slab_bytes(x6_splitk_all_plan(M, Ntot, K), M, Ntot);
  return (need > all ? need : all) + 256;
}

extern "C" int64_t gct_linear_dgrad_ws_bytes(int64_t M, int Ntot, int K) {
  int64_t m1 = 0;
  const int s = x6_tail_plan(M, K, Ntot, &m1);
  const int64_t tail = slab_bytes(s, M - m1, K);
  const int64_t all = slab_bytes(x6_splitk_all_plan(M, K, Ntot), M, K);
  return (tail > all ? tail : all) + 256;
}

extern "C" int gct_linear_dgrad(const float* dy0, const float* dy1, const float* dy2, int64_t lddy,
                                int64_t M, int nseg, int nper, const float* w0, const float* w1,
                                const float* w2, int64_t ldw, const uint16_t* wp0,
                                int64_t plane_stride, int K, float* dx, int64_t lddx, int depi,
                                const float* pre, float p, uint64_t seed, uint32_t site,
                                float* ws, int64_t ws_bytes, const int32_t* quad_map, int64_t pre_rows,
                                void* stream) {
  GCT_CHECK_ARG(ws_bytes >= 0, "linear_dgrad: negative workspace size");
  GCT_CHECK_ARG(dy0 && w0 && dx && M >= 0 && K > 0 && nseg >= 1 && nseg <= 3 && nper > 0,
                "linear_dgrad: bad args");
  GCT_CHECK_ARG(!quad_map || M % 4 == 0, "linear_dgrad: compacted rows come in quads");
  GCT_CHECK_ARG(nseg < 2 || (w1 && dy1), "linear_dgrad: missing segment 1");
  GCT_CHECK_ARG(nseg < 3 || (w2 && dy2), "linear_dgrad: missing segment 2");
  GCT_CHECK_ARG(depi >= GCT_DEPI_STORE && depi <= GCT_DEPI_MUL_SAVED, "linear_dgrad: unknown epilogue %d", depi);
  GCT_CHECK_ARG(depi != GCT_DEPI_GELU_BWD || pre, "linear_dgrad: GELU bwd needs pre");
  GCT_CHECK_ARG(depi != GCT_DEPI_MUL_SAVED || pre, "linear_dgrad: saved-factor epilogue needs pre");
  GCT_CHECK_ARG(p >= 0.f && p < 1.f, "linear_dgrad: dropout p out of range");
  GemmArgs g = {};
  g.M = M; g.N = K; g.K = (int64_t)nseg * nper;
  g.a = mkseg(dy0, dy1, dy2); g.lda = lddy; g.a_nper = nper;
  g.b = mkseg(w0, w1, w2); g.ldb = ldw; g.b_nper = nper;
  g.c0 = dx; g.ldc = lddx; g.c_nper = INT64_MAX / 4;
  g.ksplit = g.K; g.nsplit = 1; g.epi = EPI_D0 + depi;
  g.pre_in = pre;
  g.thr = gct_drop_threshold(p); g.keep_scale = 1.0f / (1.0f - p); g.rng = gct_rng_make(seed, site);
  g.bp0 = wp0; g.bp_stride = plane_stride;
  g.quad_map = quad_map;
  g.pre_rows = quad_map ? pre_rows : 0;
  const bool vec = al16(dy0) && al16(dy1) && al16(dy2) && al16(w0) && al16(w1) && al16(w2) &&
                   (lddy % 4 == 0) && (ldw % 4 == 0) && (nper % 4 == 0) && (K % 4 == 0);
  return launch<true, false>(g, vec, (hipStream_t)stream, ws, ws ? ws_bytes : 0);
}

extern "C" int gct_linear_wgrad(const float* dy0, const float* dy1, const float* dy2, int64_t lddy,
                                int64_t M, int nseg, int nper, const float* x, int64_t ldx, int K,
                                float* dw0, float* dw1, float* dw2, int64_t lddw, float* db0,
                                float* db1, float* db2, float* ws, const int32_t* tile_list,
                                const int32_t* tile_count, void* stream) {
  GCT_CHECK_ARG(dy0 && x && dw0 && ws && M >= 0 && K > 0 && nseg >= 1 && nseg <= 3 && nper > 0,
                "linear_wgrad: bad args");
  GCT_CHECK_ARG(nseg < 2 || (dy1 && dw1), "linear_wgrad: missing segment 1");
  GCT_CHECK_ARG(nseg < 3 || (dy2 && dw2), "linear_wgrad: missing segment 2");
  GCT_CHECK_ARG(lddw == K, "linear_wgrad: dW must be dense [nper][K]");
  hipStream_t st = (hipStream_t)stream;
  const int64_t Ntot = (int64_t)nseg * nper;
  const bool vec = al16(dy0) && al16(dy1) && al16(dy2) && al16(x) && (lddy % 4 == 0) &&
                   (ldx % 4 == 0) && (nper % 4 == 0) && (K % 4 == 0);
  GemmArgs g = {};
  g.M = Ntot; g.N = K; g.K = M;
  g.a = mkseg(dy0, dy1, dy2); g.lda = lddy; g.a_nper = nper;
  g.b = mkseg(x, nullptr, nullptr); g.ldb = ldx; g.b_nper = INT64_MAX / 4;
  g.c0 = ws; g.ldc = K; g.c_nper = INT64_MAX / 4;
  g.slab_stride = Ntot * K;
  g.ksplit = BK; g.nsplit = 1; g.epi = EPI_SLAB;
  const bool use_x6 = gemm_mode() != GCT_GEMM_F32 && x6_ok<X6_WGRAD>(g, vec);
  if (use_x6 && tile_list && tile_count) { g.kt_list = tile_list; g.kt_count = tile_count; }
  const int splits = wgrad_splits(M, Ntot, K, use_x6);
  int64_t ks = (M + splits - 1) / splits;
  ks = (ks + BK - 1) / BK * BK;
  g.ksplit = ks > 0 ? ks : BK;
  g.nsplit = (int)((M + g.ksplit - 1) / g.ksplit);
  if (g.nsplit < 1) g.nsplit = 1;
  g.epi = EPI_SLAB;
  float* bslab = nullptr;
  if (db0) {
    if (use_x6 || fast_ok<false, false>(g, vec)) {
      int64_t off = (int64_t)g.nsplit * g.slab_stride;
      off = (off + 3) / 4 * 4;
      bslab = ws + off;
      g.bias_slab = bslab;
    } else {
      int rc = gct_colsum(dy0, dy1, dy2, lddy, M, nseg, nper, db0, db1, db2, ws, st);
      if (rc) return rc;
    }
  }
  int rc = launch<false, false>(g, vec, st);
  if (rc) return rc;
  if (bslab)
    return gct_reduce_slabs_seg2(ws, g.nsplit, g.slab_stride, dw0, dw1, dw2, (int64_t)nper * K, Ntot * K, bslab, Ntot,
                                 db0, db1, db2, nper, Ntot, st);
  return gct_reduce_slabs_seg(ws, g.nsplit, g.slab_stride, dw0, dw1, dw2, (int64_t)nper * K, Ntot * K, st);
}
```

gct_plus_amd/engine.py:

```python
from __future__ import annotations

import math
import os
from typing import List, NamedTuple, Optional

import torch

from . import ops
from .flat import HANDED_SLOTS

_SEED = {"base": None, "ctr": 0}

COMPACT_BWD = os.environ.get("GCT_COMPACT_BWD", "1") != "0"
COMPACT_MAX_FRACTION = 0.85
COMPACT_KV = os.environ.get("GCT_COMPACT_KV", "1") != "0"
COMPACT_FWD = os.environ.get("GCT_COMPACT_FWD", "1") != "0"
COMPACT_ENC_KV = os.environ.get("GCT_COMPACT_ENC_KV", "1") != "0"


GRAD_NOTIFY = None


def _grads_done(module, G: "GradSink"):
    if GRAD_NOTIFY is not None:
        if ops.SIDE_ENABLED:
            ops.join_side()
        ps = list(module.parameters())
        GRAD_NOTIFY(ps, [G.out.get(p) for p in ps])


MODEL = "model"
DECODER = "decoder"
PREFILL = "prefill"
ENCODER = "encoder"


class RowMaps(NamedTuple):
    enc_keys: bool = False
    dec_keys: bool = False
    live: bool = False
    nc_lat: int = 0
    enc_rows: int = 0
    dec_rows: int = 0
    live_rows: int = 0


def plan_rows(caller, B=0, T=0, Le=0, mask_shape=None, *, loss_rows=False, trg_mask=False, get_attn=False,
              cond2dec=False, cond2lat=False, nconds=0, n_enc=0, n_dec=0, capturing=False, compact_fwd=False,
              compact_kv=False, compact_enc_kv=False) -> RowMaps:
    c2d = cond2dec and nconds > 0
    nc_lat = nconds if (not c2d and cond2lat and nconds > 0) else 0
    Td, Lk = T + (nconds if c2d else 0), Le + nc_lat
    none = RowMaps(nc_lat=nc_lat, enc_rows=B * Le, dec_rows=B * Lk, live_rows=B * Td)
    if caller == ENCODER or capturing:
        return none
    if caller == MODEL:
        if get_attn or mask_shape is None or tuple(mask_shape) != (B, 1, Le):
            return none
        mask_ok = True
    elif caller in (DECODER, PREFILL):
        mask_ok = mask_shape is not None and math.prod(mask_shape) == B * Le
    else:
        raise ValueError(f"plan_rows: unknown caller {caller!r}")
    return none._replace(
        enc_keys=bool(caller == MODEL and compact_enc_kv and n_enc > 0),
        dec_keys=bool(mask_ok and compact_kv and n_dec > 0),
        live=bool(compact_fwd and loss_rows and trg_mask and not get_attn and not c2d and n_dec > 0
                  and Td <= ops.ATTN_DIRECT_MAX_KEYS and Lk <= ops.ATTN_DIRECT_MAX_KEYS))


class RowPlan:

    def __init__(self, ek=None, dk=None, lr=None, rows=(0, 0, 0)):
        self._maps, self._rows = (ek, dk, lr), rows
        self._pending = ops.PendingReadBack(ek, dk, lr)
        self._usable = None
        self.enc_keys = self.dec_keys = self.live = None

    @staticmethod
    def usable_keys(h, rows):
        return h["nonprefix"] == 0 and h["empty"] == 0 and 0 < h["padded"] <= COMPACT_MAX_FRACTION * rows

    @staticmethod
    def usable_live(h, rows):
        return h["violations"] == 0 and h["nonprefix"] == 0 and 0 < h["padded"] <= COMPACT_MAX_FRACTION * rows

    @classmethod
    def launch(cls, caller, dec=None, src_mask=None, trg_mask=None, loss_rows=None, B=0, T=0, Le=0, n_enc=0):
        shape = None if (src_mask is None or not src_mask.is_cuda) else tuple(src_mask.shape)
        want = plan_rows(caller, B, T, Le, shape, loss_rows=loss_rows is not None, trg_mask=trg_mask is not None,
                         get_attn=getattr(dec, "get_attn", False), cond2dec=getattr(dec, "use_cond2dec", False),
                         cond2lat=getattr(dec, "use_cond2lat", False), nconds=getattr(dec, "nconds", 0), n_enc=n_enc,
                         n_dec=0 if dec is None else len(dec.layers), capturing=torch.cuda.is_current_stream_capturing(),
                         compact_fwd=COMPACT_FWD, compact_kv=COMPACT_KV, compact_enc_kv=COMPACT_ENC_KV)
        if not (want.enc_keys or want.dec_keys or want.live):
            return cls()
        ek = dk = lr = None
        if want.enc_keys or want.dec_keys:
            sm = ops.to_mask_u8(src_mask).view(B, Le)
            if want.enc_keys:
# ... 107 lines not shown
    x_in: torch.Tensor
    m1: torch.Tensor
    r1: torch.Tensor
    attn: MhaSaved
    a: torch.Tensor
    m2: torch.Tensor
    r2: torch.Tensor
    ffn: FfnSaved


class DecLayerSaved(NamedTuple):
    x: torch.Tensor
    m1: torch.Tensor
    r1: torch.Tensor
    attn_1: MhaSaved
    xa: torch.Tensor
    m2: torch.Tensor
    r2: torch.Tensor
    attn_2: MhaSaved
    xb: torch.Tensor
    m3: torch.Tensor
    r3: torch.Tensor
    ffn: FfnSaved


class EncoderSaved(NamedTuple):
    src: torch.Tensor
    econds: Optional[torch.Tensor]
    site_pe: int
    layers: List[EncLayerSaved]
    x_last: torch.Tensor
    mean: torch.Tensor
    rstd: torch.Tensor
    B: int
    L: int


class DecoderSaved(NamedTuple):
    trg: torch.Tensor
    z2: torch.Tensor
    dconds: Optional[torch.Tensor]
    site_pe: int
    layers: List[DecLayerSaved]
    x_last: torch.Tensor
    mean: torch.Tensor
    rstd: torch.Tensor
    B: int
    T: int
    Le: int
    Lk: int
    c2d: bool
    c2l: bool
    trg_mask_u8: Optional[torch.Tensor]
    keys: object
    live: object


def mha_fwd(run: Run, m, xq, xkv, B, Lq, Lk, mask_u8, resid, want_probs=False, keys=None, live=None):
    d, H = m.d_model, m.h
    dk = d // H
    self_attn = xkv is xq
    Mq = xq.shape[0]
    self_split = self_attn and keys is not None and live is None and not want_probs
    if self_split:
        xkv = keys.gather(xq)
    if self_attn and not self_split:
        qkv = _empty(Mq, 3 * d, xq)
        ops.linear_fwd(xq, [m.q_linear.weight, m.k_linear.weight, m.v_linear.weight],
                       [m.q_linear.bias, m.k_linear.bias, m.v_linear.bias],
                       [qkv, qkv[:, d:], qkv[:, 2 * d:]], 3 * d)
        q, k, v, ldq, ldkv = qkv, qkv[:, d:], qkv[:, 2 * d:], 3 * d, 3 * d
        qb, kvb = qkv, None
        if live is not None:
            keys = live
    else:
        qb = _empty(Mq, d, xq)
        ops.linear_fwd(xq, [m.q_linear.weight], [m.q_linear.bias], [qb], d)
        kvb = _empty(B * Lk, 2 * d, xkv) if keys is None else keys.empty(2 * d)
        ops.linear_fwd(xkv, [m.k_linear.weight, m.v_linear.weight],
                       [m.k_linear.bias, m.v_linear.bias], [kvb, kvb[:, d:]], 2 * d)
        q, k, v, ldq, ldkv = qb, kvb, kvb[:, d:], d, 2 * d
    site_p = run.site()
    o, lse, probs = ops.attn_fwd(q, k, v, ldq, ldkv, ldkv, mask_u8, B, H, Lq, Lk, dk, run.p,
                                 run.seed, site_p, want_probs=want_probs, keys=keys, live=live)
    y = _empty(Mq, d, xq)
    site_o = run.site()
    if resid is not None:
        ops.linear_fwd(o, [m.out.weight], [m.out.bias], [y], d, epi=ops.EPI_DROP_RESID,
                       resid=resid, p=run.p, seed=run.seed, site=site_o, live=live)
    else:
        ops.linear_fwd(o, [m.out.weight], [m.out.bias], [y], d)
    saved = MhaSaved(xq, xkv, qb, kvb, o, lse, mask_u8, B, Lq, Lk, site_p, site_o, resid is not None,
                     None if (self_attn and live is not None) else keys, self_split)
    return y, saved, probs


def mha_bwd(run: Run, m, sv: MhaSaved, dy, G: GradSink, dxq_out, depi_q, dxkv_out=None,
            depi_kv=ops.DEPI_STORE, live=None, gdrop=None):
    B, Lq, Lk, keys = sv.B, sv.Lq, sv.Lk, sv.keys
    d, H = m.d_model, m.h
    dk = d // H
    Mq, Mk = B * Lq, sv.xkv.shape[0]
    kt = run.kt
    new = lambda cols: _empty(Mq, cols, dy)
    if live is not None:
        Mq, kt = live.Mc, None
        new = live.empty_zero_gaps
        o_in, xq_in = (sv.o, sv.xq) if live.fwd else (live.gather(sv.o), live.gather(sv.xq))
    else:
        o_in, xq_in = sv.o, sv.xq
    if gdrop is not None:
        g = gdrop
    else:
        g = ops.dropout_bwd(dy, run.p, run.seed, sv.site_o, live=live) if (sv.fused and run.p > 0) else dy
    ops.linear_wgrad([g], d, o_in, [G(m.out.weight)], [G(m.out.bias)], kt=kt)
    do = _empty(Mq, d, dy) if live is None else live.empty(d)
    ops.linear_dgrad([g], d, Mq, [m.out.weight], do)
    if sv.kvb is None:
        dqkv = new(3 * d)
        fwdc = live is not None and live.fwd
        ops.attn_bwd(sv.qb, sv.qb[:, d:], sv.qb[:, 2 * d:], 3 * d, 3 * d, 3 * d, sv.mask_u8, sv.o, do, sv.lse, dqkv,
                     dqkv[:, d:], dqkv[:, 2 * d:], 3 * d, 3 * d, 3 * d, B, H, Lq, Lk, dk, run.p,
                     run.seed, sv.site_p, live=live, kv_compact=live is not None and not fwdc,
                     keys=live if fwdc else None)
        segs = [dqkv, dqkv[:, d:], dqkv[:, 2 * d:]]
        ops.linear_wgrad(segs, 3 * d, xq_in,
                         [G(m.q_linear.weight), G(m.k_linear.weight), G(m.v_linear.weight)],
                         [G(m.q_linear.bias), G(m.k_linear.bias), G(m.v_linear.bias)], kt=kt)
        ops.linear_dgrad(segs, 3 * d, Mq,
                         [m.q_linear.weight, m.k_linear.weight, m.v_linear.weight], dxq_out,
                         depi=depi_q)
    else:
        dq = new(d)
        if keys is None:
            dkv = _empty(Mk, 2 * d, dy)
        else:
            dkv = keys.empty_zero_gaps(2 * d)
        ops.attn_bwd(sv.qb, sv.kvb, sv.kvb[:, d:], d, 2 * d, 2 * d, sv.mask_u8, sv.o, do, sv.lse, dq, dkv, dkv[:, d:],
                     d, 2 * d, 2 * d, B, H, Lq, Lk, dk, run.p, run.seed, sv.site_p, live=live, keys=keys)
        ops.linear_wgrad([dq], d, xq_in, [G(m.q_linear.weight)], [G(m.q_linear.bias)], kt=kt)
        ops.linear_wgrad([dkv, dkv[:, d:]], 2 * d, sv.xkv,
                         [G(m.k_linear.weight), G(m.v_linear.weight)],
                         [G(m.k_linear.bias), G(m.v_linear.bias)])
        ops.linear_dgrad([dq], d, Mq, [m.q_linear.weight], dxq_out, depi=depi_q)
        if sv.self_split:
            dxk = keys.empty(d)
            ops.linear_dgrad([dkv, dkv[:, d:]], 2 * d, Mk, [m.k_linear.weight, m.v_linear.weight], dxk)
            keys.scatter_add(dxk, dxq_out)
        elif dxkv_out is not None:
            ops.linear_dgrad([dkv, dkv[:, d:]], 2 * d, Mk, [m.k_linear.weight, m.v_linear.weight],
                             dxkv_out, depi=depi_kv)


def ffn_fwd(run: Run, ff, x, resid, live=None):
    M, d = x.shape
    dff = ff.linear_1.weight.shape[0]
    gelu_d = _empty(M, dff, x)
    hdn = _empty(M, dff, x)
    site_h = run.site()
    ops.linear_fwd(x, [ff.linear_1.weight], [ff.linear_1.bias], [hdn], dff, epi=ops.EPI_GELU_DROP_SAVE,
                   pre=gelu_d, p=run.p, seed=run.seed, site=site_h, live=live)
    y = _empty(M, d, x)
    site_o = run.site()
    if resid is not None:
        ops.linear_fwd(hdn, [ff.linear_2.weight], [ff.linear_2.bias], [y], d,
                       epi=ops.EPI_DROP_RESID, resid=resid, p=run.p, seed=run.seed, site=site_o, live=live)
    else:
        ops.linear_fwd(hdn, [ff.linear_2.weight], [ff.linear_2.bias], [y], d)
    return y, FfnSaved(x, gelu_d, hdn, site_h, site_o, resid is not None)


def ffn_bwd(run: Run, ff, sv: FfnSaved, dy, G: GradSink, dx_out, depi, live=None, gdrop=None):
    x, gelu_d, hdn = sv.x, sv.gelu_d, sv.hdn
    M, d = x.shape
    dff = gelu_d.shape[1]
    kt = run.kt
    if live is not None:
        M, kt = live.Mc, None
        if not live.fwd:
            x, hdn = live.gather(x), live.gather(hdn)
    if gdrop is not None:
        g = gdrop
    else:
        g = ops.dropout_bwd(dy, run.p, run.seed, sv.site_o, live=live) if (sv.fused and run.p > 0) else dy
    ops.linear_wgrad([g], d, hdn, [G(ff.linear_2.weight)], [G(ff.linear_2.bias)], kt=kt)
    dpre = _empty(M, dff, dy) if live is None else live.empty(dff)
    ops.linear_dgrad([g], d, M, [ff.linear_2.weight], dpre, depi=ops.DEPI_MUL_SAVED, pre=gelu_d,
                     p=run.p, seed=run.seed, site=sv.site_h, live=live, pre_full=live is not None and not live.fwd)
    ops.linear_wgrad([dpre], dff, x, [G(ff.linear_1.weight)], [G(ff.linear_1.bias)], kt=kt)
    ops.linear_dgrad([dpre], dff, M, [ff.linear_1.weight], dx_out, depi=depi)


def enc_layer_fwd(run: Run, layer, x_in, B, L, mask_u8, want_probs=False, keys=None):
    n1, m1, r1 = ops.norm_fwd(x_in, layer.norm_1.alpha, layer.norm_1.bias, layer.norm_1.eps)
    a, sv_a, probs = mha_fwd(run, layer.attn, n1, n1, B, L, L, mask_u8, n1, want_probs, keys=keys)
    n2, m2, r2 = ops.norm_fwd(a, layer.norm_2.alpha, layer.norm_2.bias, layer.norm_2.eps)
    out, sv_f = ffn_fwd(run, layer.ff, n2, n2)
    return out, EncLayerSaved(x_in, m1, r1, sv_a, a, m2, r2, sv_f), probs


def _mha_drop(run: Run, sv: MhaSaved, buf):
    return (buf, run.p, run.seed, sv.site_o) if (buf is not None and sv.fused and run.p > 0) else None


def _ffn_drop(run: Run, sv: Optional[FfnSaved], buf):
    return (buf, run.p, run.seed, sv.site_o) if (buf is not None and sv is not None and sv.fused and run.p > 0) else None


def enc_layer_bwd(run: Run, layer, sv: EncLayerSaved, g, G: GradSink, gd=None, gdbuf=None, below=None):
    with ops.deferred_reductions():
        ffn_bwd(run, layer.ff, sv.ffn, g, G, g, ops.DEPI_ACCUM, gdrop=gd)
        dr = _mha_drop(run, sv.attn, gdbuf)
        ops.norm_bwd(g, sv.a, layer.norm_2.alpha, sv.m2, sv.r2, G(layer.norm_2.alpha), G(layer.norm_2.bias),
                     out=g, eps=layer.norm_2.eps, drop=dr)
        mha_bwd(run, layer.attn, sv.attn, g, G, g, ops.DEPI_ACCUM, gdrop=None if dr is None else gdbuf)
        dr = _ffn_drop(run, below, gdbuf)
        ops.norm_bwd(g, sv.x_in, layer.norm_1.alpha, sv.m1, sv.r1, G(layer.norm_1.alpha), G(layer.norm_1.bias),
                     out=g, eps=layer.norm_1.eps, drop=dr)
    _grads_done(layer, G)
    return g, (None if dr is None else gdbuf)


def dec_layer_fwd(run: Run, layer, x, e, B, T, Lk, src_mask_u8, trg_mask_u8, want_probs=False, keys=None, live=None):
    x2, m1, r1 = ops.norm_fwd(x, layer.norm_1.alpha, layer.norm_1.bias, layer.norm_1.eps)
    xa, sa1, p1 = mha_fwd(run, layer.attn_1, x2, x2, B, T, T, trg_mask_u8, x, want_probs, live=live)
    x2, m2, r2 = ops.norm_fwd(xa, layer.norm_2.alpha, layer.norm_2.bias, layer.norm_2.eps)
    xb, sa2, p2 = mha_fwd(run, layer.attn_2, x2, e, B, T, Lk, src_mask_u8, xa, want_probs, keys=keys, live=live)
    x2, m3, r3 = ops.norm_fwd(xb, layer.norm_3.alpha, layer.norm_3.bias, layer.norm_3.eps)
    xc, sf = ffn_fwd(run, layer.ff, x2, xb, live=live)
    return xc, DecLayerSaved(x, m1, r1, sa1, xa, m2, r2, sa2, xb, m3, r3, sf), p1, p2


def dec_layer_bwd(run: Run, layer, sv: DecLayerSaved, g, de, first_de, G: GradSink, live=None, gd=None, gdbuf=None,
                  below=None):
    t = torch.empty_like(g) if live is None else live.empty(g.shape[1])
    with ops.deferred_reductions():
        ffn_bwd(run, layer.ff, sv.ffn, g, G, t, ops.DEPI_STORE, live=live, gdrop=gd)
        dr = _mha_drop(run, sv.attn_2, gdbuf)
        ops.norm_bwd(t, sv.xb, layer.norm_3.alpha, sv.m3, sv.r3, G(layer.norm_3.alpha), G(layer.norm_3.bias),
                     dres=g, out=g, eps=layer.norm_3.eps, live=live, drop=dr)
        mha_bwd(run, layer.attn_2, sv.attn_2, g, G, t, ops.DEPI_STORE, de,
                ops.DEPI_STORE if first_de else ops.DEPI_ACCUM, live=live, gdrop=None if dr is None else gdbuf)
        dr = _mha_drop(run, sv.attn_1, gdbuf)
        ops.norm_bwd(t, sv.xa, layer.norm_2.alpha, sv.m2, sv.r2, G(layer.norm_2.alpha), G(layer.norm_2.bias),
                     dres=g, out=g, eps=layer.norm_2.eps, live=live, drop=dr)
        mha_bwd(run, layer.attn_1, sv.attn_1, g, G, t, ops.DEPI_STORE, live=live, gdrop=None if dr is None else gdbuf)
        dr = _ffn_drop(run, below, gdbuf)
        ops.norm_bwd(t, sv.x, layer.norm_1.alpha, sv.m1, sv.r1, G(layer.norm_1.alpha), G(layer.norm_1.bias),
                     dres=g, out=g, eps=layer.norm_1.eps, live=live, drop=dr)
    _grads_done(layer, G)
    return g, (None if dr is None else gdbuf)


def _pe2d(pe_mod, L):
    pe = pe_mod.pe
    if L > pe.shape[1]:
        raise ValueError(f"sequence length {L} exceeds the positional table ({pe.shape[1]})")
    return pe[0]


def encoder_trunk_fwd(enc, run: Run, src, mask_u8, econds, want_probs, plan: RowPlan):
    keys = plan.enc_keys
    B, S = src.shape
    d, nc = enc.d_model, enc.nconds
    cond = None
    if nc > 0:
        if econds is None:
            raise ValueError("econds required when nconds > 0")
        cond = ops.small_linear_fwd(econds.contiguous(), enc.embed_cond2enc.weight,
                                    enc.embed_cond2enc.bias)
    L = S + nc
    mask_u8 = ops.pack_mask(mask_u8, B, L, L)
    site_pe = run.site()
    x = ops.embed_pe_fwd(src, enc.embed_sentence.embed.weight, cond, _pe2d(enc.pe, L), nc,
                         math.sqrt(d), run.p, run.seed, site_pe)
    layers, probs = [], []
    for layer in enc.layers:
        x, sv, pr = enc_layer_fwd(run, layer, x, B, L, mask_u8, want_probs, keys=keys)
        layers.append(sv)
        probs.append(pr)
    y, mean, rstd = ops.norm_fwd(x, enc.norm.alpha, enc.norm.bias, enc.norm.eps)
    return y.view(B, L, d), EncoderSaved(src, econds, site_pe, layers, x, mean, rstd, B, L), probs


def encoder_trunk_bwd(enc, run: Run, sv: EncoderSaved, dy, G: GradSink):
    layers, B, L = sv.layers, sv.B, sv.L
    d, nc = enc.d_model, enc.nconds
    g = dy.reshape(B * L, d).clone()
    gdbuf = torch.empty_like(g) if (run.p > 0 and len(layers) > 0) else None
    dr = _ffn_drop(run, layers[-1].ffn if layers else None, gdbuf)
    ops.norm_bwd(g, sv.x_last, enc.norm.alpha, sv.mean, sv.rstd, G(enc.norm.alpha), G(enc.norm.bias), out=g,
                 eps=enc.norm.eps, drop=dr)
    gd = None if dr is None else gdbuf
    for i in range(len(layers) - 1, -1, -1):
        g, gd = enc_layer_bwd(run, enc.layers[i], layers[i], g, G, gd=gd, gdbuf=gdbuf,
                              below=layers[i - 1].ffn if i > 0 else None)
    dcond = torch.empty(B, nc * d, dtype=torch.float32, device=g.device) if nc > 0 else None
    ops.embed_pe_bwd(g, sv.src, G(enc.embed_sentence.embed.weight), dcond, nc, math.sqrt(d), run.p,
                     run.seed, sv.site_pe)
    if nc > 0:
        ops.small_linear_bwd(dcond, sv.econds.contiguous(), G(enc.embed_cond2enc.weight),
                             G(enc.embed_cond2enc.bias))


def decoder_trunk_fwd(dec, run: Run, trg, z, src_mask_u8, trg_mask_u8, dconds, want_probs, plan: RowPlan):
    B, T0 = trg.shape
    d, nc = dec.d_model, dec.nconds
    Le, lat = z.shape[1], z.shape[2]
    z2 = z.reshape(B * Le, lat)
    c2d = dec.use_cond2dec and nc > 0
    c2l = (not c2d) and dec.use_cond2lat and nc > 0
    cond_x = None
    if c2d:
        cond_x = ops.small_linear_fwd(dconds.contiguous(), dec.embed_cond2dec.weight,
                                      dec.embed_cond2dec.bias)
    T = T0 + (nc if c2d else 0)
    site_pe = run.site()
    x = ops.embed_pe_fwd(trg, dec.embed.embed.weight, cond_x, _pe2d(dec.pe, T), nc if c2d else 0,
                         math.sqrt(d), run.p, run.seed, site_pe)
    ez = _empty(B * Le, d, z2)
    ops.linear_fwd(z2, [dec.fc_z.weight], [dec.fc_z.bias], [ez], d)
    Lk = Le
    e = ez
    if c2l:
        Lk = Le + nc
        cl = ops.small_linear_fwd(dconds.contiguous(), dec.embed_cond2lat.weight,
                                  dec.embed_cond2lat.bias)
        e = _empty(B * Lk, d, z2)
        ops.copy_rows(cl, nc, 0, e, Lk, 0, B * nc, nc, d)
        ops.copy_rows(ez, Le, 0, e, Lk, nc, B * Le, Le, d)
        if src_mask_u8 is not None:
            ones = torch.ones(B, nc, dtype=torch.uint8, device=src_mask_u8.device)
            src_mask_u8 = torch.cat([ones, src_mask_u8.view(B, Le)], dim=1).contiguous()
    layers, p1s, p2s = [], [], []
    live, keys = plan.live, plan.dec_keys
    if live is not None:
        x = live.gather(x)
    if keys is not None:
        e = keys.gather(e)
    src_m = ops.pack_mask(src_mask_u8, B, T, Lk)
    trg_m = ops.pack_mask(trg_mask_u8, B, T, T)
    for layer in dec.layers:
        x, sv, p1, p2 = dec_layer_fwd(run, layer, x, e, B, T, Lk, src_m, trg_m, want_probs, keys=keys, live=live)
        layers.append(sv)
        p1s.append(p1)
        p2s.append(p2)
    y, mean, rstd = ops.norm_fwd(x, dec.norm.alpha, dec.norm.bias, dec.norm.eps)
    saved = DecoderSaved(trg, z2, dconds, site_pe, layers, x, mean, rstd, B, T, Le, Lk, c2d, c2l,
                         trg_mask_u8.u8 if isinstance(trg_mask_u8, ops.MaskBits) else trg_mask_u8, keys, live)
    if live is not None:
        return y, saved, p1s, p2s
    return y.view(B, T, d), saved, p1s, p2s


def decoder_trunk_bwd(dec, run: Run, sv: DecoderSaved, dy, G: GradSink, need_dz=True):
    layers, keys, live_fwd = sv.layers, sv.keys, sv.live
    B, T, Le, Lk = sv.B, sv.T, sv.Le, sv.Lk
    new_de = (lambda: _empty(B * Lk, d, dy)) if keys is None else (lambda: keys.empty(d))
    d, nc = dec.d_model, dec.nconds
    live, lr = live_fwd, None
    if live_fwd is None:
        lr = ops.LiveRows(dy.reshape(B * T, d), B, T, sv.trg_mask_u8) if (COMPACT_BWD or (B * T) % 32 == 0) else None
        if COMPACT_BWD and len(dec.layers) > 0 and not torch.cuda.is_current_stream_capturing():
            live = lr if RowPlan.usable_live(lr.host(), B * T) else None
    if live_fwd is not None:
        g = dy.reshape(live.Mc, d).clone()
    elif live is not None:
        g = live.gather(dy.reshape(B * T, d))
    else:
        g = dy.reshape(B * T, d).clone()
        run.kt = lr.kt if (lr is not None and (B * T) % 32 == 0) else None
    gdbuf = None
    if run.p > 0 and len(layers) > 0:
        gdbuf = torch.empty_like(g) if live is None else live.empty(d)
    dr = _ffn_drop(run, layers[-1].ffn if layers else None, gdbuf)
    ops.norm_bwd(g, sv.x_last, dec.norm.alpha, sv.mean, sv.rstd, G(dec.norm.alpha), G(dec.norm.bias), out=g,
                 eps=dec.norm.eps, live=live, drop=dr)
    gd = None if dr is None else gdbuf
    de = new_de()
    for i in range(len(layers) - 1, -1, -1):
        g, gd = dec_layer_bwd(run, dec.layers[i], layers[i], g, de, i == len(layers) - 1, G, live=live, gd=gd,
                              gdbuf=gdbuf, below=layers[i - 1].ffn if i > 0 else None)
    run.kt = None
    if live is not None:
        g = live.scatter(g)
    if len(dec.layers) == 0:
        de.zero_()
    if keys is not None:
        de = keys.scatter(de)
    dcx = torch.empty(B, nc * d, dtype=torch.float32, device=g.device) if sv.c2d else None
    ops.embed_pe_bwd(g, sv.trg, G(dec.embed.embed.weight), dcx, nc if sv.c2d else 0, math.sqrt(d), run.p,
                     run.seed, sv.site_pe)
    if sv.c2d:
        ops.small_linear_bwd(dcx, sv.dconds.contiguous(), G(dec.embed_cond2dec.weight),
                             G(dec.embed_cond2dec.bias))
    dez = de
    if sv.c2l:
        dcl = torch.empty(B, nc * d, dtype=torch.float32, device=g.device)
        ops.copy_rows(de, Lk, 0, dcl, nc, 0, B * nc, nc, d)
        ops.small_linear_bwd(dcl, sv.dconds.contiguous(), G(dec.embed_cond2lat.weight),
                             G(dec.embed_cond2lat.bias))
        dez = _empty(B * Le, d, g)
        ops.copy_rows(de, Lk, nc, dez, Le, 0, B * Le, Le, d)
    ops.linear_wgrad([dez], d, sv.z2, [G(dec.fc_z.weight)], [G(dec.fc_z.bias)])
    dz = None
    if need_dz:
        dz = _empty(B * Le, sv.z2.shape[1], g)
        ops.linear_dgrad([dez], d, B * Le, [dec.fc_z.weight], dz)
        dz = dz.view(B, Le, -1)
    return dz


def _f32c(t):
    return t if (t.dtype == torch.float32 and t.is_contiguous()) else t.float().contiguous()


class EncoderFn(torch.autograd.Function):
    @staticmethod
    def forward(ctx, enc, run, src, mask_u8, econds, want_probs, plan, *params):
        y, saved, probs = encoder_trunk_fwd(enc, run, src, mask_u8, econds, want_probs, plan)
        ctx.enc, ctx.run, ctx.saved, ctx.params = enc, run, saved, params
        if want_probs:
            for p in probs:
                ctx.mark_non_differentiable(p)
            return (y, *probs)
        return y

    @staticmethod
    def backward(ctx, dy, *unused):
        G = GradSink()
        encoder_trunk_bwd(ctx.enc, ctx.run, ctx.saved, _f32c(dy), G)
        ctx.saved = None
        return (None,) * 7 + G.collect(ctx.params)


class DecoderFn(torch.autograd.Function):
    @staticmethod
    def forward(ctx, dec, run, trg, z, src_mask_u8, trg_mask_u8, dconds, want_probs, plan, *params):
        y, saved, p1, p2 = decoder_trunk_fwd(dec, run, trg, _f32c(z), src_mask_u8, trg_mask_u8, dconds, want_probs,
                                             plan)
        ctx.dec, ctx.run, ctx.saved, ctx.params = dec, run, saved, params
        ctx.need_dz = z.requires_grad
        if want_probs:
            for p in p1 + p2:
                ctx.mark_non_differentiable(p)
            return (y, *p1, *p2)
        return y

    @staticmethod
    def backward(ctx, dy, *unused):
        G = GradSink()
        dz = decoder_trunk_bwd(ctx.dec, ctx.run, ctx.saved, _f32c(dy), G, ctx.need_dz)
        ctx.saved = None
        return (None, None, None, dz, None, None, None, None, None) + G.collect(ctx.params)


class ScatterRowsFn(torch.autograd.Function):

    @staticmethod
# ... 290 lines not shown
```

gct_plus_amd/ops.py:

```python
from __future__ import annotations

import contextlib
import math
import os
import threading
import weakref
from typing import List, Optional, Sequence

import torch

from . import _lib
from ._lib import check

EPI_BIAS, EPI_GELU_DROP, EPI_DROP_RESID, EPI_GELU_DROP_SAVE = 0, 1, 2, 3
DEPI_STORE, DEPI_ACCUM, DEPI_GELU_BWD, DEPI_MUL_SAVED = 0, 1, 2, 3


def _L():
    return _lib.load()


_raw_stream, _cur_dev = torch._C._cuda_getCurrentRawStream, torch._C._cuda_getDevice


def _st():
    return _raw_stream(_cur_dev())


def _p(t: Optional[torch.Tensor]):
    return None if t is None else t.data_ptr()


def _chk(t: torch.Tensor, name: str, dtype=torch.float32):
    if not t.is_cuda:
        raise _lib.GctError(f"{name}: expected a CUDA (ROCm) tensor; gct_plus_amd has no CPU path")
    if t.dtype != dtype:
        raise _lib.GctError(f"{name}: expected {dtype}, got {t.dtype}")
    return t


SIDE_ENABLED = os.environ.get("GCT_SIDE_STREAM", "0") != "0"
_SIDE = {}
_PENDING = {}


def _side_stream(device):
    idx = device.index if device.index is not None else torch.cuda.current_device()
    st = _SIDE.get(idx)
    if st is None:
        st = torch.cuda.Stream(device=idx)
        _SIDE[idx] = st
    return st


def _wait_pending(t):
    if _PENDING and t is not None:
        ev = _PENDING.pop(t.untyped_storage().data_ptr(), None)
        if ev is not None:
            torch.cuda.current_stream().wait_event(ev)


def join_side(device=None):
    if _SIDE:
        cur = torch.cuda.current_stream()
        for st in _SIDE.values():
            cur.wait_stream(st)
        _PENDING.clear()


_WS = {}


def workspace(nbytes: int, device) -> torch.Tensor:
    key = (device.index if device.index is not None else torch.cuda.current_device(), _st())
    buf = _WS.get(key)
    if buf is None or buf.numel() * 4 < nbytes:
        n = max(int(nbytes * 1.25) // 4 + 64, 1 << 20)
        buf = torch.empty(n, dtype=torch.float32, device=device)
        _WS[key] = buf
    return buf


DEFER_REDUCTIONS = os.environ.get("GCT_DEFER_REDUCTIONS", "1") != "0"
class _DeferState(threading.local):
    def __init__(self):
        self.d = {"on": False, "off": 0, "demand": 0, "want": 0}


_DEFER_TL = _DeferState()
_ARENA = {}


def kept_workspace(nbytes: int, device) -> torch.Tensor:
    if not _DEFER_TL.d["on"]:
        return workspace(nbytes, device)
    key = (device.index if device.index is not None else torch.cuda.current_device(), _st())
    n = (int(nbytes) + 255) // 256 * 64
    _DEFER_TL.d["demand"] += n
# ... 145 lines not shown
def gemm_x3_launches() -> int:
    return int(_L().gct_gemm_x3_launches())


def gemm_launch_counts():
    import ctypes
    out = (ctypes.c_int64 * 2)()
    check(_L().gct_gemm_launch_counts(ctypes.cast(out, ctypes.c_void_p)), "gct_gemm_launch_counts")
    return int(out[0]), int(out[1])


def split_planes(flat: torch.Tensor, planes: Optional[torch.Tensor] = None) -> torch.Tensor:
    _chk(flat, "flat")
    n = flat.numel()
    if planes is None:
        planes = torch.empty(3, n, dtype=torch.int16, device=flat.device)
    check(_L().gct_split_planes(_p(flat), n, _p(planes), planes.stride(0), _st()), "gct_split_planes")
    return planes


def _drop_planes(base: int, end: int):
    _PLANES[:] = [e for e in _PLANES if e[1] <= base or e[0] >= end]


def register_planes(flat: torch.Tensor, planes: torch.Tensor):
    base, end = flat.data_ptr(), flat.data_ptr() + flat.numel() * 4
    known = any(e[0] == base and e[1] == end and e[4]() is flat for e in _PLANES)
    _drop_planes(base, end)
    _PLANES.append((base, end, planes, flat.numel(), weakref.ref(flat)))
    if not known:
        weakref.finalize(flat, _drop_planes, base, end)


def unregister_planes(flat: torch.Tensor):
    _drop_planes(flat.data_ptr(), flat.data_ptr() + flat.numel() * 4)


def _plane_ptr(ws_):
    if not _PLANES:
        return None, 0
    a = ws_[0].data_ptr()
    for base, end, planes, numel, ref in _PLANES:
        if base <= a < end:
            if ref() is None:
                return None, 0
            if all(base <= w.data_ptr() < end for w in ws_[1:]):
                return planes.data_ptr() + (a - base) // 2, planes.stride(0)
            return None, 0
    return None, 0


def linear_fwd(x2d, ws_: Sequence[torch.Tensor], bs: Sequence[Optional[torch.Tensor]],
               outs: Sequence[torch.Tensor], ldy: int, epi=EPI_BIAS, resid=None, pre=None,
               p=0.0, seed=0, site=0, splitk_ws: Optional[torch.Tensor] = None, ws: Optional[torch.Tensor] = None,
               live=None):
    M, K = x2d.shape
    nper = ws_[0].shape[0]
    w = _seg3(ws_)
    b = _seg3(bs)
    y = _seg3(outs)
    need = _ws_need("gct_linear_fwd_ws_bytes", M, K, nper * len(ws_))
    for t in (splitk_ws, ws):
        if t is not None and t.numel() * 4 < need:
            raise _lib.GctError(f"linear_fwd: workspace of {t.numel() * 4} B < {need} B "
                                f"(gct_linear_fwd_ws_bytes({M}, {K}, {nper * len(ws_)}))")
    if splitk_ws is not None:
        wp, pstride, wsb, quad_map, timed = None, 0, splitk_ws, None, contextlib.nullcontext()
    else:
        wp, pstride = _plane_ptr(ws_)
        wsb = ws if ws is not None else (workspace(need, x2d.device) if need > 256 else None)
        quad_map = None if live is None else _p(live.quad_list)
        N = nper * len(ws_)
        nbytes = 4 * M * K + (6 if wp else 4) * N * K + 4 * N + 4 * M * N * (2 if epi in (EPI_GELU_DROP, EPI_DROP_RESID, EPI_GELU_DROP_SAVE) else 1)
        timed = _Timed("gemm_fwd", 2.0 * M * K * N, nbytes)
    with timed:
        check(_L().gct_linear_fwd(_p(x2d), x2d.stride(0), M, K, w[0], w[1], w[2], ws_[0].stride(0),
                                  wp, pstride, b[0], b[1], b[2], len(ws_), nper, y[0], y[1], y[2],
                                  ldy, epi, _p(resid), _p(pre), p, seed, site, _p(wsb),
                                  0 if wsb is None else wsb.numel() * 4, quad_map, _st()),
              "gct_linear_fwd")


def linear_dgrad(dys: Sequence[torch.Tensor], lddy: int, M: int, ws_: Sequence[torch.Tensor], dx,
                 depi=DEPI_STORE, pre=None, p=0.0, seed=0, site=0, live=None, pre_full=False):
    nper, K = ws_[0].shape
    d = _seg3(dys)
    w = _seg3(ws_)
    _wait_pending(dx)
    with _Timed("gemm_dgrad", 2.0 * M * K * nper * len(ws_)):
        wp, pstride = _plane_ptr(ws_)
        need = _ws_need("gct_linear_dgrad_ws_bytes", M, nper * len(ws_), K)
        wsb = workspace(need, dx.device) if need > 256 else None
        check(_L().gct_linear_dgrad(d[0], d[1], d[2], lddy, M, len(ws_), nper, w[0], w[1], w[2],
                                    ws_[0].stride(0), wp, pstride, K, _p(dx), dx.stride(0), depi,
                                    _p(pre), p, seed, site, _p(wsb), 0 if wsb is None else wsb.numel() * 4,
                                    None if live is None else _p(live.quad_list),
                                    pre.shape[0] if (live is not None and pre is not None and pre_full) else 0,
                                    _st()), "gct_linear_dgrad")


def nonzero_row_tiles(x2d: torch.Tensor):
    _chk(x2d, "x2d")
    rows, cols = x2d.shape
    nt = (rows + 31) // 32
    lst = torch.empty(max(nt, 1), dtype=torch.int32, device=x2d.device)
    cnt = torch.empty(1, dtype=torch.int32, device=x2d.device)
    flags = torch.empty(max(nt, 1), dtype=torch.uint8, device=x2d.device)
    check(_L().gct_nonzero_row_tiles(_p(x2d), x2d.stride(0), rows, cols, _p(lst), _p(cnt), _p(flags), _st()),
          "gct_nonzero_row_tiles")
    return lst, cnt


_SKIPPED = {}
_SKIPPED_MSG = ("{} decoder rows that an earlier forward skipped (loss_rows: rows that do not reach the loss) received a "
                "non-zero gradient in its backward pass: that gradient was ignored, and the optimizer steps launched since "
                "then were skipped on the device (FusedAdam's guard), so no wrong update has been applied; this error is "
                "raised at the first host read-back after the fact.  Call the model without loss_rows "
                "(forward_propagation(..., skip_ignored=False)) for losses other than the reference's ignore_index "
                "cross-entropy.")


def assert_no_skipped_row_gradients():
    n = int(skipped_row_gradients().item())
    if n:
        skipped_row_gradients().zero_()
        raise _lib.GctError(_SKIPPED_MSG.format(n))


def skipped_row_gradients():
    dev = torch.cuda.current_device()
    t = _SKIPPED.get(dev)
    if t is None:
        t = _SKIPPED[dev] = torch.zeros(1, dtype=torch.int32, device=torch.device("cuda", dev))
    return t


class LiveRows:
    SLACK = 256
    fwd = False

    def __init__(self, g2d, B, T, mask_u8, lists=True):
        _chk(g2d, "g2d")
        dev = g2d.device
        M = B * T
        assert g2d.shape[0] == M
        nt, nq = (M + 31) // 32, (M + 3) // 4
        i32 = lambda n: torch.empty(max(n, 1), dtype=torch.int32, device=dev)
        self.B, self.T, self.M, self.dev = B, T, M, dev
        self.live = torch.empty(max(M, 1), dtype=torch.uint8, device=dev)
        self.n_b, self.info = i32(B), i32(8)
        self.cstart = i32(B) if lists else None
        self.quad_list = i32(nq + 32) if lists else None
        qrank = i32(nq) if lists else None
        self.tile_list, self.tile_count = i32(nt), i32(1)
        flags = torch.empty(max(nt, 1), dtype=torch.uint8, device=dev)
        if mask_u8 is None:
            sb = sq = 0
        else:
            _chk(mask_u8, "live_rows.mask", torch.uint8)
            sb, sq = _mask_strides(mask_u8, B, T, T)
        check(_L().gct_live_rows(_p(g2d), g2d.stride(0), B, T, g2d.shape[1], _p(mask_u8), sb, sq, _p(self.live),
                                 _p(self.n_b), _p(self.info), _p(self.cstart), _p(self.quad_list), _p(qrank),
                                 _p(self.tile_list), _p(self.tile_count), _p(flags), _st()), "gct_live_rows")
        self.kt = (self.tile_list, self.tile_count)
        self._host = None
        self.Mc = None

    @classmethod
    def from_rows(cls, rows_u8, B, T, mask_u8):
        _chk(rows_u8, "live_rows.rows", torch.uint8)
        return cls(rows_u8.reshape(B * T, 1).to(torch.float32), B, T, mask_u8)

    def _fill_host(self, v):
        self._host = dict(n_live=v[0], violations=v[1], nonprefix=v[2], tiles=v[3], padded=v[4], quads=v[5], empty=v[6])
        self.Mc = v[4]

    def host(self):
        if self._host is None:
            PendingReadBack(self).finish()
        return self._host

# ... 95 lines not shown
    d = _seg3(dys)
    dw = _seg3(dws)
    db = _seg3(dbs)

    def launch():
        ws = kept_workspace(_ws_need("gct_wgrad_ws_bytes", M, nseg * nper, K), x2d.device)
        with _Timed("gemm_wgrad+bias+reduce", 2.0 * M * K * nper * nseg):
            check(_L().gct_linear_wgrad(d[0], d[1], d[2], lddy, M, nseg, nper, _p(x2d), x2d.stride(0),
                                        K, dw[0], dw[1], dw[2], K, db[0], db[1], db[2], _p(ws),
                                        _p(kt[0]) if kt else None, _p(kt[1]) if kt else None, _st()),
                  "gct_linear_wgrad")

    if not SIDE_ENABLED or torch.cuda.is_current_stream_capturing():
        launch()
        return
    main = torch.cuda.current_stream()
    side = _side_stream(x2d.device)
    ready = torch.cuda.Event()
    ready.record(main)
    side.wait_event(ready)
    with torch.cuda.stream(side):
        launch()
        done = torch.cuda.Event()
        done.record(side)
    for t in list(dys) + [x2d]:
        t.record_stream(side)
        _PENDING[t.untyped_storage().data_ptr()] = done


def dropout_bwd(dout2d, p, seed, site, out=None, live=None):
    rows, cols = dout2d.shape
    if live is not None:
        rows = live.Mc
    dy = torch.empty_like(dout2d) if out is None else out
    _wait_pending(out)
    check(_L().gct_dropout_bwd(_p(dout2d), _p(dy), rows, cols, p, seed, site,
                               None if live is None else _p(live.quad_list), _st()), "gct_dropout_bwd")
    return dy


ATTN_DIRECT_MAX_KEYS = 96


class MaskBits:

    def __init__(self, mask_u8, B, Lq, Lk):
        _chk(mask_u8, "attn.mask", torch.uint8)
        if Lk > 256 or Lq > 256:
            raise _lib.GctError(f"attention: sequence length {max(Lq, Lk)} > 256 unsupported")
        sb, sq = _mask_strides(mask_u8, B, Lq, Lk)
        rows = 1 if sq == 0 else Lq
        self.u8, self.B, self.Lq, self.Lk = mask_u8, B, Lq, Lk
        self.bits = torch.empty(B, rows, 8, dtype=torch.int32, device=mask_u8.device)
        self.sb, self.sq = rows * 8, (0 if sq == 0 else 8)
        ntr = 1 if sq == 0 else (Lq + 15) // 16
        self.tiles = torch.empty(B, ntr, dtype=torch.int32, device=mask_u8.device)
        self.t_sb, self.t_su = ntr, (0 if sq == 0 else 1)
        check(_L().gct_attn_mask_pack(_p(mask_u8), sb, sq, B, Lq, Lk, _p(self.bits), _p(self.tiles), _st()),
              "gct_attn_mask_pack")


def pack_mask(mask, B, Lq, Lk) -> Optional["MaskBits"]:
    if mask is None or isinstance(mask, MaskBits):
        if isinstance(mask, MaskBits) and (mask.B, mask.Lk) != (B, Lk):
            raise _lib.GctError(f"packed mask was built for B={mask.B}, Lk={mask.Lk}, not B={B}, Lk={Lk}")
        return mask
    return MaskBits(to_mask_u8(mask), B, Lq, Lk)


def _mb(mask, B, Lq, Lk):
    mb = pack_mask(mask, B, Lq, Lk)
    if mb is None:
        return None, 0, 0, None
    if mb.t_su and mb.Lq != Lq:
        raise _lib.GctError(f"packed mask was built for Lq={mb.Lq}, not Lq={Lq}")
    return mb.bits.data_ptr(), mb.sb, mb.sq, mb


def _tb(mb):
    return (None, 0, 0) if mb is None else (mb.tiles.data_ptr(), mb.t_sb, mb.t_su)


def attn_fwd(q, k, v, ld_q, ld_k, ld_v, mask, B, H, Lq, Lk, dk, p, seed, site, out=None,
             want_probs=False, keys=None, live=None):
    dev = q.device
    if out is not None:
        o = out
    elif live is not None:
        o = live.empty_zero_gaps(H * dk)
    else:
        o = torch.empty(B * Lq, H * dk, dtype=torch.float32, device=dev)
    lse = torch.empty(B * H * Lq, dtype=torch.float32, device=dev)
    probs = torch.empty(B, H, Lq, Lk, dtype=torch.float32, device=dev) if want_probs else None
    mp, sb, sq, mask_owner = _mb(mask, B, Lq, Lk)
    check(_L().gct_attn_fwd(_p(q), ld_q, _p(k), ld_k, _p(v), ld_v, mp, sb, sq, _p(o),
                            o.stride(0), _p(lse), _p(probs), B, H, Lq, Lk, dk,
                            1.0 / math.sqrt(dk), p, seed, site, None if keys is None else _p(keys.cstart),
                            None if keys is None else _p(keys.n_b), *_tb(mask_owner),
                            None if live is None else _p(live.cstart), None if live is None else _p(live.n_b),
                            _st()), "gct_attn_fwd")
    del mask_owner
    return o, lse, probs


_ATTN_BWD_WS = {}


def _attn_bwd_ws(dev, nbytes):
    if nbytes <= 0:
        return None
    key = (dev, _st())
    ws = _ATTN_BWD_WS.get(key)
    if ws is None or ws.numel() < nbytes:
        ws = torch.empty(nbytes, dtype=torch.uint8, device=dev)
        _ATTN_BWD_WS[key] = ws
    return ws


def attn_bwd(q, k, v, ld_q, ld_k, ld_v, mask, o, dout, lse, dq, dk_, dv, ld_dq, ld_dk, ld_dv,
             B, H, Lq, Lk, dk, p, seed, site, live=None, kv_compact=False, keys=None):
    ws = _attn_bwd_ws(q.device, int(_L().gct_attn_bwd_ws_bytes(B, H, Lq, Lk)))
    mp, sb, sq, mask_owner = _mb(mask, B, Lq, Lk)
    check(_L().gct_attn_bwd(_p(q), ld_q, _p(k), ld_k, _p(v), ld_v, mp, sb, sq, _p(o),
                            _p(dout), o.stride(0), _p(lse), _p(dq), ld_dq, _p(dk_), ld_dk,
                            _p(dv), ld_dv, B, H, Lq, Lk, dk, 1.0 / math.sqrt(dk), p, seed, site,
                            None if live is None else _p(live.cstart), None if live is None else _p(live.n_b),
                            int(bool(kv_compact)) | (2 if (live is not None and live.fwd) else 0),
                            None if keys is None else _p(keys.cstart),
                            None if keys is None else _p(keys.n_b), *_tb(mask_owner), _p(ws),
                            0 if ws is None else ws.numel(),
                            _st()), "gct_attn_bwd")
    del mask_owner


def _mask_strides(mask_u8, B, Lq, Lk):
    if mask_u8 is None:
        return 0, 0
    _chk(mask_u8, "attn.mask", torch.uint8)
    n = mask_u8.numel()
    if n == B * Lk:
        return Lk, 0
    if n == B * Lq * Lk:
        return Lq * Lk, Lk
    raise _lib.GctError(f"attention mask with {n} elements fits neither [B,Lk] nor [B,Lq,Lk] "
                        f"(B={B}, Lq={Lq}, Lk={Lk})")


def trg_mask_u8(target: torch.Tensor, pad_id: int) -> torch.Tensor:
    _chk(target, "trg_mask.target", torch.int64)
    B, T = target.shape
    out = torch.empty(B, T, T, dtype=torch.uint8, device=target.device)
    check(_L().gct_trg_mask_tokens(_p(target), target.stride(0), int(pad_id), B, T, _p(out), _st()),
          "gct_trg_mask_tokens")
    return out


def to_mask_u8(mask: Optional[torch.Tensor]) -> Optional[torch.Tensor]:
    if mask is None:
        return None
    if mask.dtype == torch.uint8:
        return mask.contiguous()
    return (mask != 0).to(torch.uint8).contiguous()


def reparam_fwd(mu, log_var, eps, seed, site):
    z = torch.empty_like(mu)
    eps_out = torch.empty_like(mu)
    check(_L().gct_reparam_fwd(_p(mu), _p(log_var), _p(eps), _p(eps_out), _p(z), mu.numel(), seed,
                               site, _st()), "gct_reparam_fwd")
    return z, eps_out


def reparam_bwd(dz, log_var, eps, dmu_ext, dlv_ext, dmu, dlv):
    check(_L().gct_reparam_bwd(_p(dz), _p(log_var), _p(eps), _p(dmu_ext), _p(dlv_ext), _p(dmu),
                               _p(dlv), dz.numel(), _st()), "gct_reparam_bwd")


def kld_fwd(mu, log_var):
    out = torch.empty((), dtype=torch.float32, device=mu.device)
    ws = workspace(4096, mu.device)
    check(_L().gct_kld_fwd(_p(mu), _p(log_var), _p(out), _p(ws), mu.numel(), _st()), "gct_kld_fwd")
    return out


def kld_bwd(mu, log_var, gout):
    dmu, dlv = torch.empty_like(mu), torch.empty_like(log_var)
    check(_L().gct_kld_bwd(_p(mu), _p(log_var), _p(gout), _p(dmu), _p(dlv), mu.numel(), _st()),
          "gct_kld_bwd")
    return dmu, dlv


def ce_fwd(logits2d, target, pad_id):
    _chk(target, "ce.target", torch.int64)
    rows, V = logits2d.shape
    out = torch.empty((), dtype=torch.float32, device=logits2d.device)
    ws = workspace(4096, logits2d.device)
    check(_L().gct_ce_fwd(_p(logits2d), _p(target), _p(out), _p(ws), rows, V, pad_id, _st()),
          "gct_ce_fwd")
    return out


def ce_bwd(logits2d, target, gout, pad_id):
    rows, V = logits2d.shape
    dl = torch.empty_like(logits2d)
    check(_L().gct_ce_bwd(_p(logits2d), _p(target), _p(gout), _p(dl), rows, V, pad_id, _st()),
          "gct_ce_bwd")
    return dl


def adam_step(p, g, m, v, lr, b1, b2, eps, step, gscale=1.0, guard=True):
    check(_L().gct_adam_step(_p(p), _p(g), _p(m), _p(v), p.numel(), lr, b1, b2, eps, step, gscale,
                             _p(skipped_row_gradients()) if guard else None, _st()), "gct_adam_step")


# ... 156 lines not shown
```

include/gctplus_hip.h:

```cpp
#ifndef GCTPLUS_HIP_H
#define GCTPLUS_HIP_H

#include <stdint.h>

#ifdef __cplusplus
extern "C" {
#endif

#define GCT_OK 0
#define GCT_ERR_ARG (-1)
#define GCT_ERR_HIP (-2)

#define GCT_ABI_VERSION 20

int gct_version(void);
const char* gct_last_error(void);

int64_t gct_wgrad_ws_bytes(int64_t M, int64_t Ntot, int64_t K);
int64_t gct_rowred_ws_bytes(int64_t rows, int64_t cols);

int gct_norm_fwd(const float* x, const float* alpha, const float* bias, float* y,
                 float* mean, float* rstd, int64_t rows, int d, float eps, void* stream);
int gct_norm_bwd(const float* dy, const float* x, const float* alpha, const float* mean,
                 const float* rstd, const float* dres, float* dx, float* dalpha, float* dbias,
                 float* ws, int64_t rows, int d, float eps, const int32_t* quad_map, int64_t src_rows,
                 float* drop_out, float p, uint64_t seed, uint32_t site, void* stream);

int gct_embed_pe_fwd(const int64_t* tok, const float* table, const float* cond, const float* pe,
                     float* out, int B, int S, int n_c, int d, int vocab, float scale, float p,
                     uint64_t seed, uint32_t site, void* stream);
int64_t gct_embed_ws_bytes(int B, int S, int d, int vocab);
int gct_embed_pe_bwd(const float* dout, const int64_t* tok, float* dtable, float* dcond,
                     float* ws, int B, int S, int n_c, int d, int vocab, float scale, float p,
                     uint64_t seed, uint32_t site, void* stream);

#define GCT_EPI_BIAS 0
#define GCT_EPI_GELU_DROP 1
#define GCT_EPI_DROP_RESID 2
#define GCT_EPI_GELU_DROP_SAVE 3
int gct_linear_fwd(const float* x, int64_t ldx, int64_t M, int K,
                   const float* w0, const float* w1, const float* w2, int64_t ldw,
                   const uint16_t* wp0, int64_t plane_stride,
                   const float* b0, const float* b1, const float* b2,
                   int nseg, int nper, float* y0, float* y1, float* y2, int64_t ldy,
                   int epi, const float* resid, float* pre, float p, uint64_t seed, uint32_t site,
                   float* ws, int64_t ws_bytes, const int32_t* quad_map, void* stream);
int64_t gct_linear_fwd_ws_bytes(int64_t M, int K, int Ntot);

#define GCT_DEPI_STORE 0
#define GCT_DEPI_ACCUM 1
#define GCT_DEPI_GELU_BWD 2
#define GCT_DEPI_MUL_SAVED 3
int gct_linear_dgrad(const float* dy0, const float* dy1, const float* dy2, int64_t lddy,
                     int64_t M, int nseg, int nper,
                     const float* w0, const float* w1, const float* w2, int64_t ldw,
                     const uint16_t* wp0, int64_t plane_stride, int K,
                     float* dx, int64_t lddx, int depi, const float* pre, float p, uint64_t seed,
                     uint32_t site, float* ws, int64_t ws_bytes, const int32_t* quad_map, int64_t pre_rows,
                     void* stream);
int64_t gct_linear_dgrad_ws_bytes(int64_t M, int Ntot, int K);

int gct_linear_wgrad(const float* dy0, const float* dy1, const float* dy2, int64_t lddy,
                     int64_t M, int nseg, int nper, const float* x, int64_t ldx, int K,
                     float* dw0, float* dw1, float* dw2, int64_t lddw,
                     float* db0, float* db1, float* db2, float* ws,
                     const int32_t* tile_list, const int32_t* tile_count, void* stream);

#define GCT_GEMM_F32 0
#define GCT_GEMM_BF16X6 1
#define GCT_GEMM_BF16X3 2
int gct_gemm_set_mode(int mode);
int gct_gemm_get_mode(void);
int gct_gemm_launch_counts(int64_t* out2);
int64_t gct_gemm_x6_kernel_launches(void);
int64_t gct_gemm_x3_launches(void);

int gct_split_planes(const float* src, int64_t numel, uint16_t* planes, int64_t plane_stride,
                     void* stream);

int gct_dead_rows_nonzero(const float* g, int64_t ld, int64_t rows, int cols, const uint8_t* live,
                          int32_t* counter, void* stream);
int gct_nonzero_row_tiles(const float* x, int64_t ld, int64_t rows, int cols, int32_t* list,
                          int32_t* count, uint8_t* flags_ws, void* stream);
int gct_live_rows(const float* g, int64_t ld, int B, int T, int cols, const uint8_t* mask, int64_t mask_sb,
                  int64_t mask_sq, uint8_t* live, int32_t* n_b, int32_t* info, int32_t* cstart,
                  int32_t* quad_list, int32_t* qrank_ws, int32_t* tile_list, int32_t* tile_count,
                  uint8_t* tile_flags_ws, void* stream);
int gct_key_rows(const uint8_t* mask, int64_t mask_sb, int B, int Lk, uint8_t* live, int32_t* n_b, int32_t* info,
                 int32_t* cstart, int32_t* quad_list, int32_t* qrank_ws, void* stream);
int gct_gather_quads(const float* src, int64_t ld, int64_t M, const int32_t* quad_list, int64_t nrows, int cols,
                     float* dst, int64_t ldd, void* stream);
int gct_scatter_quads(const float* src, int64_t ld, const int32_t* quad_list, int64_t nrows, int cols, float* dst,
                      int64_t ldd, int64_t M, void* stream);
int gct_zero_gap_rows(float* buf, int64_t ld, int cols, const int32_t* cstart, const int32_t* n_b, int B, int64_t nrows,
                      void* stream);
int gct_scatter_add_quads(const float* src, int64_t ld, const int32_t* quad_list, int64_t nrows, int cols, float* dst,
                          int64_t ldd, int64_t M, void* stream);

int gct_dropout_bwd(const float* dout, float* dy, int64_t rows, int cols, float p, uint64_t seed,
                    uint32_t site, const int32_t* quad_map, void* stream);

#define GCT_ATTN_DIRECT_MAX_KEYS 96
int gct_attn_mask_pack(const uint8_t* mask, int64_t mask_sb, int64_t mask_sq, int B, int Lq, int Lk,
                       uint32_t* bits, uint32_t* tiles, void* stream);
int gct_trg_mask_tokens(const int64_t* tokens, int64_t ld_tok, int64_t pad, int B, int T, uint8_t* out, void* stream);
int gct_attn_fwd(const float* q, int64_t ldq, const float* k, int64_t ldk, const float* v,
                 int64_t ldv, const uint32_t* mbits, int64_t mb_sb, int64_t mb_sq,
                 float* o, int64_t ldo, float* lse, float* probs, int B, int H, int Lq, int Lk,
                 int dk, float scale, float p, uint64_t seed, uint32_t site, const int32_t* kstart,
                 const int32_t* klen, const uint32_t* tbits, int64_t tb_sb, int64_t tb_su,
                 const int32_t* qstart, const int32_t* qlen, void* stream);
int gct_attn_bwd(const float* q, int64_t ldq, const float* k, int64_t ldk, const float* v,
                 int64_t ldv, const uint32_t* mbits, int64_t mb_sb, int64_t mb_sq,
                 const float* o, const float* dout, int64_t ldo, const float* lse,
                 float* dq, int64_t lddq, float* dk_, int64_t lddk, float* dv, int64_t lddv,
                 int B, int H, int Lq, int Lk, int dk, float scale, float p, uint64_t seed,
                 uint32_t site, const int32_t* cstart, const int32_t* nlive, int kv_compact,
                 const int32_t* kstart, const int32_t* klen, const uint32_t* tbits, int64_t tb_sb, int64_t tb_su,
                 void* ws, int64_t ws_bytes, void* stream);
int64_t gct_attn_bwd_ws_bytes(int B, int H, int Lq, int Lk);

int gct_reparam_fwd(const float* mu, const float* log_var, const float* eps_in, float* eps_out,
                    float* z, int64_t n, uint64_t seed, uint32_t site, void* stream);
int gct_reparam_bwd(const float* dz, const float* log_var, const float* eps, const float* dmu_ext,
                    const float* dlv_ext, float* dmu, float* dlv, int64_t n, void* stream);
int gct_kld_fwd(const float* mu, const float* log_var, float* out, float* ws, int64_t n,
                void* stream);
int gct_kld_bwd(const float* mu, const float* log_var, const float* gout, float* dmu, float* dlv,
                int64_t n, void* stream);

int gct_ce_fwd(const float* logits, const int64_t* target, float* out, float* ws, int64_t rows,
               int V, int64_t pad_id, void* stream);
int gct_ce_bwd(const float* logits, const int64_t* target, const float* gout, float* dlogits,
               int64_t rows, int V, int64_t pad_id, void* stream);

int gct_adam_step(float* p, const float* g, float* m, float* v, int64_t n, float lr, float b1,
                  float b2, float eps, int64_t step, float gscale, const int32_t* skip_if_nonzero,
                  void* stream);

int gct_attn_decode(const float* q, int64_t ldq, float* k, float* v, int64_t kv_row,
                    int64_t kv_batch, const uint8_t* valid, int64_t valid_sb, float* o, int64_t ldo,
                    int n, int H, int Lc, int dk, float scale, const int32_t* pos, int cache_off,
                    const float* knew, const float* vnew, int64_t ldn, const int32_t* klen,
                    const int32_t* row_off, void* stream);
int gct_attn_decode_z(const float* q, int64_t ldq, int qoff, const float* z, int64_t z_batch, int lat, int Le,
                      const float* ckv, int64_t ckv_batch, int64_t ld_ckv, int nc, const uint8_t* valid,
                      int64_t valid_sb, const int32_t* klen, float* out, int64_t ldo, int ooff, int n, int H, int dk,
                      float scale, void* stream);
int gct_decode_embed(const int64_t* ys, int64_t ld_ys, const int32_t* pos, int pe_off, const float* table,
                     int vocab, const float* pe, float* out, int n, int d, float scale, const int32_t* row_off,
                     void* stream);
int gct_decode_advance(int32_t* pos, void* stream);
typedef struct GctSampleFilter {
  int32_t k;
  float top_p;
  float inv_temp;
  int32_t reserved;
} GctSampleFilter;
#define GCT_SAMPLE_FILTER_MAX_VOCAB 1024
int gct_select_token(const float* logits, int V, int64_t* ys, int64_t ld_ys, int pos, uint8_t* valid,
                     int64_t valid_sb, uint8_t* done, float* probs_out, int n, int mode,
                     int64_t pad_id, int64_t eos_id, uint64_t seed, const int32_t* pos_dev, int valid_off,
                     const uint64_t* seed_dev, const int32_t* row_off, const GctSampleFilter* filt,
                     const int32_t* item, const int32_t* prefix_len, int item_base, void* stream);

#define GCT_STREAM_MAX_ROWS 8192
#define GCT_STREAM_MAX_LAYERS 16
typedef struct GctStreamState {
  int64_t* ys;
  uint8_t* valid;
  uint8_t* done;
  int32_t* row_off;
  const int32_t* pos;
  float* z3;
  uint8_t* src_valid;
  int32_t* src_klen;
  float* ckv[GCT_STREAM_MAX_LAYERS];
  int32_t* item;
  int32_t* harvest;
  uint8_t* fresh;
  const float* z_pool;
  const uint8_t* valid_pool;
  const int32_t* klen_pool;
  const float* ckv_pool[GCT_STREAM_MAX_LAYERS];
  const int64_t* prefix_pool;
  const int32_t* prefix_len;
  const int32_t* limit;
  int64_t* out_ys;
  int32_t* out_len;
  int32_t* row_of;
  int32_t* start_step;
  int32_t* next_item;
  int32_t* n_harvested;
  const int32_t* enable;
  int64_t rows, items, ld_ys, valid_sb, valid_off, T, width, t0_max, z_row, Lk, ckv_row, layers, pad_id;
} GctStreamState;
int gct_stream_refill(const GctStreamState* state, void* stream);

#define GCT_BEAM_MAX_K 16
#define GCT_BEAM_MAX_VOCAB 65536
int gct_attn_decode_beam(const float* q, int64_t ldq, float* k, float* v, int64_t kv_row, int64_t kv_batch,
                         const uint8_t* valid, int64_t valid_sb, float* o, int64_t ldo, int n, int H, int T, int dk,
                         float scale, const int32_t* pos, int cache_off, const float* knew, const float* vnew,
// ... 32 lines not shown
```

Measured before the change: 11110.

## Fold gap-row zeroing into attention kernels and scatter-accumulate into dgrad epilogue

```diff
diff --git a/gct_plus_amd/csrc/attention.hip b/gct_plus_amd/csrc/attention.hip
--- a/gct_plus_amd/csrc/attention.hip
+++ b/gct_plus_amd/csrc/attention.hip
@@ -30,6 +30,7 @@
   int kv_compact;
   int qo_compact;
   const int32_t *kstart, *klen;
+  int q_rows, kv_rows;
   float4* ws_meta;
   uint32_t* ws_keep;
   uint32_t* ws_use;
@@ -407,8 +408,26 @@
   }
 }
 
+template <int DK>
+__device__ __forceinline__ void zero_head_rows(float* buf, int ld, int h, int64_t r0, int64_t r1, int lane) {
+  constexpr int C = DK / 4, RPI = 64 / C;
+  const int c = lane % C;
+  for (int64_t r = r0 + lane / C; r < r1; r += RPI)
+    *reinterpret_cast<float4*>(buf + r * ld + h * DK + 4 * c) = make_float4(0.f, 0.f, 0.f, 0.f);
+}
+__device__ __forceinline__ int gap_owner_tile(int n) { return n > 0 ? (n - 1) >> 4 : 0; }
+template <int DK>
+__device__ __forceinline__ void zero_gap_share(float* buf, int ld, int h, const int32_t* start, const int32_t* len, int b,
+                                               int B, int rows, int lane) {
+  const int64_t t0 = (int64_t)start[B - 1] + len[B - 1];
+  const int64_t g0 = (int64_t)start[b] + len[b], g1 = b + 1 < B ? (int64_t)start[b + 1] : t0;
+  zero_head_rows<DK>(buf, ld, h, g0, g1 < rows ? g1 : rows, lane);
+  const int64_t per = (rows - t0 + B - 1) / B, s0 = t0 + b * per, s1 = s0 + per;
+  if (per > 0) zero_head_rows<DK>(buf, ld, h, s0, s1 < rows ? s1 : rows, lane);
+}
+
 template <int NDT, int NT>
-__global__ __launch_bounds__(256, 6) void attn_fwd_direct_kernel(const AttnArgs a) {
+__global__ __launch_bounds__(256, 7) void attn_fwd_direct_kernel(const AttnArgs a) {
   constexpr int DK = 16 * NDT, MW = mask_words(NT);
   typedef typename VecN<NDT>::T VT;
   const int lane = threadIdx.x & 63, g = lane >> 4, c16 = lane & 15;
@@ -421,6 +440,8 @@
   const int q = 16 * u + c16;
   const int Lq_e = a.qo_compact ? a.nlive[b] : a.Lq;
   const int64_t qr0 = a.qo_compact ? (int64_t)a.cstart[b] : (int64_t)b * a.Lq;
+  if (a.q_rows > 0 && u == gap_owner_tile(Lq_e))
+    zero_gap_share<DK>(a.o, a.ldo, h, a.cstart, a.nlive, b, a.B, a.q_rows, (int)__lane_id());
   if (16 * u >= Lq_e) return;
   const int Lk_in = a.klen ? a.klen[b] : a.Lk;
   const int64_t kr0 = a.kstart ? (int64_t)a.kstart[b] : (int64_t)b * a.Lk;
@@ -848,6 +869,8 @@
   const int Lk_in = a.klen ? a.klen[b] : a.Lk;
   const int klast = Lk_in > 0 ? Lk_in - 1 : 0;
   uint32_t* visit = a.ws_use + (int64_t)pair * nqt + u;
+  if (a.q_rows > 0 && u == gap_owner_tile(Lq_e))
+    zero_gap_share<DK>(a.dq, a.lddq, h, a.cstart, a.nlive, b, a.B, a.q_rows, lane);
   if (16 * u >= Lq_e) {
     if (lane == 0) *visit = 0;
     return;
@@ -1010,6 +1033,11 @@
   const int Lk_in = a.klen ? a.klen[b] : a.Lk;
   const int Lk_e = a.kv_compact ? Lq_e : Lk_in;
   const int64_t krow0 = a.kv_compact ? drow0 : kin0;
+  if (a.kv_rows > 0 && t == gap_owner_tile(Lk_e)) {
+    const int32_t *st = a.kv_compact ? a.cstart : a.kstart, *ln = a.kv_compact ? a.nlive : a.klen;
+    zero_gap_share<DK>(a.dk, a.lddk, h, st, ln, b, a.B, a.kv_rows, lane);
+    zero_gap_share<DK>(a.dv, a.lddv, h, st, ln, b, a.B, a.kv_rows, lane);
+  }
   if (16 * t >= Lk_e) return;
   const int k = 16 * t + c16;
   const bool inr = k < a.Lk;
@@ -1369,12 +1397,13 @@
   return GCT_OK;
 }
 
-extern "C" int gct_attn_fwd(const float* q, int64_t ldq, const float* k, int64_t ldk,
-                            const float* v, int64_t ldv, const uint32_t* mbits, int64_t mb_sb,
-                            int64_t mb_sq, float* o, int64_t ldo, float* lse, float* probs, int B,
-                            int H, int Lq, int Lk, int dk, float scale, float p, uint64_t seed,
-                            uint32_t site, const int32_t* kstart, const int32_t* klen, const uint32_t* tbits,
-                            int64_t tb_sb, int64_t tb_su, const int32_t* qstart, const int32_t* qlen, void* stream) {
+extern "C" int gct_attn_fwd_gaps(const float* q, int64_t ldq, const float* k, int64_t ldk,
+                                 const float* v, int64_t ldv, const uint32_t* mbits, int64_t mb_sb,
+                                 int64_t mb_sq, float* o, int64_t ldo, float* lse, float* probs, int B,
+                                 int H, int Lq, int Lk, int dk, float scale, float p, uint64_t seed,
+                                 uint32_t site, const int32_t* kstart, const int32_t* klen, const uint32_t* tbits,
+                                 int64_t tb_sb, int64_t tb_su, const int32_t* qstart, const int32_t* qlen,
+                                 int64_t q_rows, void* stream) {
   int rc = check_common("attn_fwd", q, ldq, k, ldk, v, ldv, mbits, mb_sb, mb_sq, B, H, Lq, Lk, dk, p);
   if (rc) return rc;
   GCT_CHECK_ARG(o && lse && ldo % 4 == 0 && gct_aligned16(o) && (int64_t)Lq * ldo * 4 < (1ll << 31), "attn_fwd: bad output");
@@ -1394,6 +1423,9 @@
                 "attn_fwd: compact query rows need the direct kernel (Lk <= %d) and no probs output",
                 GCT_ATTN_DIRECT_MAX_KEYS);
   a.cstart = qstart; a.nlive = qlen; a.qo_compact = qstart ? 1 : 0;
+  GCT_CHECK_ARG(q_rows >= 0 && q_rows <= INT32_MAX && (q_rows == 0 || qstart),
+                "attn_fwd: q_rows (zero the gap rows of o) needs compact query rows");
+  a.q_rows = (int)q_rows;
   a.B = B; a.H = H; a.Lq = Lq; a.Lk = Lk; a.npairs = B * H; a.scale = scale;
   a.thr = gct_drop_threshold(p); a.keep_scale = 1.0f / (1.0f - p); a.rng = gct_rng_make(seed, site);
   rc = launch<false>(dk, plan_attn_fwd(Lq, Lk, dk, a.npairs, num_cus()), a, (hipStream_t)stream);
@@ -1402,20 +1434,31 @@
   return GCT_OK;
 }
 
+extern "C" int gct_attn_fwd(const float* q, int64_t ldq, const float* k, int64_t ldk,
+                            const float* v, int64_t ldv, const uint32_t* mbits, int64_t mb_sb,
+                            int64_t mb_sq, float* o, int64_t ldo, float* lse, float* probs, int B,
+                            int H, int Lq, int Lk, int dk, float scale, float p, uint64_t seed,
+                            uint32_t site, const int32_t* kstart, const int32_t* klen, const uint32_t* tbits,
+                            int64_t tb_sb, int64_t tb_su, const int32_t* qstart, const int32_t* qlen, void* stream) {
+  return gct_attn_fwd_gaps(q, ldq, k, ldk, v, ldv, mbits, mb_sb, mb_sq, o, ldo, lse, probs, B, H, Lq, Lk, dk, scale, p,
+                           seed, site, kstart, klen, tbits, tb_sb, tb_su, qstart, qlen, 0, stream);
+}
+
 extern "C" int64_t gct_attn_bwd_ws_bytes(int B, int H, int Lq, int Lk) {
   if (B <= 0 || H <= 0 || Lq <= 0 || Lk <= 0 || Lk > GCT_ATTN_DIRECT_MAX_KEYS) return 0;
   return bwd_ws_layout(B, H, Lq).bytes;
 }
 
-extern "C" int gct_attn_bwd(const float* q, int64_t ldq, const float* k, int64_t ldk,
-                            const float* v, int64_t ldv, const uint32_t* mbits, int64_t mb_sb,
-                            int64_t mb_sq, const float* o, const float* dout, int64_t ldo,
-                            const float* lse, float* dq, int64_t lddq, float* dk_,
-                            int64_t lddk, float* dv, int64_t lddv, int B, int H, int Lq, int Lk,
-                            int dk, float scale, float p, uint64_t seed, uint32_t site,
-                            const int32_t* cstart, const int32_t* nlive, int kv_compact,
-                            const int32_t* kstart, const int32_t* klen, const uint32_t* tbits, int64_t tb_sb,
-                            int64_t tb_su, void* ws, int64_t ws_bytes, void* stream) {
+extern "C" int gct_attn_bwd_gaps(const float* q, int64_t ldq, const float* k, int64_t ldk,
+                                 const float* v, int64_t ldv, const uint32_t* mbits, int64_t mb_sb,
+                                 int64_t mb_sq, const float* o, const float* dout, int64_t ldo,
+                                 const float* lse, float* dq, int64_t lddq, float* dk_,
+                                 int64_t lddk, float* dv, int64_t lddv, int B, int H, int Lq, int Lk,
+                                 int dk, float scale, float p, uint64_t seed, uint32_t site,
+                                 const int32_t* cstart, const int32_t* nlive, int kv_compact,
+                                 const int32_t* kstart, const int32_t* klen, const uint32_t* tbits, int64_t tb_sb,
+                                 int64_t tb_su, void* ws, int64_t ws_bytes, int64_t q_rows, int64_t kv_rows,
+                                 void* stream) {
   int rc = check_common("attn_bwd", q, ldq, k, ldk, v, ldv, mbits, mb_sb, mb_sq, B, H, Lq, Lk, dk, p);
   if (rc) return rc;
   GCT_CHECK_ARG(o && dout && lse && dq && dk_ && dv, "attn_bwd: null pointer");
@@ -1446,6 +1489,12 @@
   a.kstart = kstart; a.klen = klen;
   GCT_CHECK_ARG(!qo_compact || Lk <= GCT_ATTN_DIRECT_MAX_KEYS,
                 "attn_bwd: compact q / o rows need the direct kernels (Lk <= %d)", GCT_ATTN_DIRECT_MAX_KEYS);
+  GCT_CHECK_ARG(q_rows >= 0 && q_rows <= INT32_MAX && kv_rows >= 0 && kv_rows <= INT32_MAX &&
+                    (q_rows == 0 || cstart) && (kv_rows == 0 || kv_compact || kstart) &&
+                    ((q_rows == 0 && kv_rows == 0) || Lk <= GCT_ATTN_DIRECT_MAX_KEYS),
+                "attn_bwd: q_rows / kv_rows (zero the gap rows of dq / dk, dv) need compact rows on that side and the "
+                "direct kernels (Lk <= %d)", GCT_ATTN_DIRECT_MAX_KEYS);
+  a.q_rows = (int)q_rows; a.kv_rows = (int)kv_rows;
   const int64_t ws_need = gct_attn_bwd_ws_bytes(B, H, Lq, Lk);
   GCT_CHECK_ARG(ws_need == 0 || (ws && gct_aligned16(ws) && ws_bytes >= ws_need),
                 "attn_bwd: Lk <= %d needs a 16-B aligned workspace of %lld B (gct_attn_bwd_ws_bytes); got %lld B at %p",
@@ -1465,3 +1514,17 @@
   GCT_LAUNCH_CHECK("attn_bwd");
   return GCT_OK;
 }
+
+extern "C" int gct_attn_bwd(const float* q, int64_t ldq, const float* k, int64_t ldk,
+                            const float* v, int64_t ldv, const uint32_t* mbits, int64_t mb_sb,
+                            int64_t mb_sq, const float* o, const float* dout, int64_t ldo,
+                            const float* lse, float* dq, int64_t lddq, float* dk_,
+                            int64_t lddk, float* dv, int64_t lddv, int B, int H, int Lq, int Lk,
+                            int dk, float scale, float p, uint64_t seed, uint32_t site,
+                            const int32_t* cstart, const int32_t* nlive, int kv_compact,
+                            const int32_t* kstart, const int32_t* klen, const uint32_t* tbits, int64_t tb_sb,
+                            int64_t tb_su, void* ws, int64_t ws_bytes, void* stream) {
+  return gct_attn_bwd_gaps(q, ldq, k, ldk, v, ldv, mbits, mb_sb, mb_sq, o, dout, ldo, lse, dq, lddq, dk_, lddk, dv, lddv,
+                           B, H, Lq, Lk, dk, scale, p, seed, site, cstart, nlive, kv_compact, kstart, klen, tbits, tb_sb,
+                           tb_su, ws, ws_bytes, 0, 0, stream);
+}
diff --git a/gct_plus_amd/csrc/gemm.hip b/gct_plus_amd/csrc/gemm.hip
--- a/gct_plus_amd/csrc/gemm.hip
+++ b/gct_plus_amd/csrc/gemm.hip
@@ -346,7 +346,12 @@
           const int64_t row = row_base + e;
           if (row >= g.M) continue;
           float v = acc[i][j][q4 * 4 + e];
-          const int64_t off = row * g.ldc + cloc;
+          int64_t off = row * g.ldc + cloc;
+          if (g.epi == EPI_D0 + GCT_DEPI_ACCUM_MAPPED) {
+            const int64_t er0 = pre_row0(g, row_base);
+            if (er0 < 0 || er0 + e >= g.pre_rows) continue;
+            off = (er0 + e) * g.ldc + cloc;
+          }
           const bool keep = gct_drop_keep(bits, e, (uint32_t)col, g.thr);
           switch (g.epi) {
             case GCT_EPI_BIAS:
@@ -370,6 +375,7 @@
               v += g.resid[off];
             } break;
             case EPI_D0 + GCT_DEPI_ACCUM:
+            case EPI_D0 + GCT_DEPI_ACCUM_MAPPED:
               v += cbase[off];
               break;
             case EPI_D0 + GCT_DEPI_GELU_BWD: {
@@ -425,8 +431,9 @@
 #ifdef GCT_LAB_NO_EPI_MATH
     return false;
 #endif
-    return (FWD && g.epi == GCT_EPI_DROP_RESID) || (BWD && g.epi == EPI_D0 + GCT_DEPI_ACCUM) || reads_pre();
-  }
+    return (FWD && g.epi == GCT_EPI_DROP_RESID) || (BWD && g.epi == EPI_D0 + GCT_DEPI_ACCUM) || maps_out() || reads_pre();
+  }
+  __device__ __forceinline__ bool maps_out() const { return BWD && g.epi == EPI_D0 + GCT_DEPI_ACCUM_MAPPED; }
   __device__ __forceinline__ bool reads_pre() const {
     return BWD && (g.epi == EPI_D0 + GCT_DEPI_GELU_BWD || g.epi == EPI_D0 + GCT_DEPI_MUL_SAVED);
   }
@@ -437,7 +444,7 @@
                                            int64_t cloc) const {
     const float* eb = extra_base(cbase);
     int64_t er0 = row0, elim = g.M;
-    if (reads_pre() && g.pre_rows > 0) {
+    if ((reads_pre() && g.pre_rows > 0) || maps_out()) {
       er0 = pre_row0(g, row0);
       elim = er0 < 0 ? -1 : g.pre_rows;
     }
@@ -469,11 +476,16 @@
       for (int cp = 0; cp < 2; ++cp)
         bits[cp] = gct_drop_bits(g.rng, drop_quad(g, row0), (uint32_t)(col0 + 2 * cp));
     }
+    int64_t orow0 = row0, olim = g.M;
+    if (maps_out()) {
+      orow0 = pre_row0(g, row0);
+      olim = orow0 < 0 ? -1 : g.pre_rows;
+    }
 #pragma unroll
     for (int rr = 0; rr < 4; ++rr) {
       const int64_t row = row0 + rr;
-      if (row >= g.M) break;
-      const int64_t off = row * g.ldc + cloc;
+      if (row >= g.M || orow0 + rr >= olim) break;
+      const int64_t off = (orow0 + rr) * g.ldc + cloc;
       float x[4] = {v[rr].x, v[rr].y, v[rr].z, v[rr].w};
       const float bs[4] = {bias.x, bias.y, bias.z, bias.w};
       bool keep[4] = {true, true, true, true};
@@ -506,7 +518,7 @@
 #pragma unroll
         for (int cc = 0; cc < 4; ++cc)
           x[cc] = (keep[cc] ? (x[cc] + bs[cc]) * g.keep_scale : 0.f) + rs[cc];
-      } else if (BWD && epi == EPI_D0 + GCT_DEPI_ACCUM) {
+      } else if (BWD && (epi == EPI_D0 + GCT_DEPI_ACCUM || epi == EPI_D0 + GCT_DEPI_ACCUM_MAPPED)) {
         const float4 r = ex[rr];
         x[0] += r.x; x[1] += r.y; x[2] += r.z; x[3] += r.w;
       } else if (BWD && epi == EPI_D0 + GCT_DEPI_GELU_BWD) {
@@ -1175,7 +1187,7 @@
   GemmArgs e = g;
   e.M = m2; e.row_base = g.row_base + m1;
   e.a.p0 += m1 * g.lda;
-  e.c0 += m1 * g.ldc;
+  if (g.epi != EPI_D0 + GCT_DEPI_ACCUM_MAPPED) e.c0 += m1 * g.ldc;
   if (e.resid) e.resid += m1 * g.ldc;
   if (e.pre) e.pre += m1 * g.ldc;
   if (e.pre_in && !(g.pre_rows > 0 && g.quad_map)) e.pre_in += m1 * g.ldc;
@@ -1445,7 +1457,9 @@
   GCT_CHECK_ARG(!quad_map || M % 4 == 0, "linear_dgrad: compacted rows come in quads");
   GCT_CHECK_ARG(nseg < 2 || (w1 && dy1), "linear_dgrad: missing segment 1");
   GCT_CHECK_ARG(nseg < 3 || (w2 && dy2), "linear_dgrad: missing segment 2");
-  GCT_CHECK_ARG(depi >= GCT_DEPI_STORE && depi <= GCT_DEPI_MUL_SAVED, "linear_dgrad: unknown epilogue %d", depi);
+  GCT_CHECK_ARG(depi >= GCT_DEPI_STORE && depi <= GCT_DEPI_ACCUM_MAPPED, "linear_dgrad: unknown epilogue %d", depi);
+  GCT_CHECK_ARG(depi != GCT_DEPI_ACCUM_MAPPED || (quad_map && pre_rows > 0 && !pre),
+                "linear_dgrad: the mapped accumulate needs quad_map and the rows of dx (pre_rows), and no pre");
   GCT_CHECK_ARG(depi != GCT_DEPI_GELU_BWD || pre, "linear_dgrad: GELU bwd needs pre");
   GCT_CHECK_ARG(depi != GCT_DEPI_MUL_SAVED || pre, "linear_dgrad: saved-factor epilogue needs pre");
   GCT_CHECK_ARG(p >= 0.f && p < 1.f, "linear_dgrad: dropout p out of range");
diff --git a/gct_plus_amd/engine.py b/gct_plus_amd/engine.py
--- a/gct_plus_amd/engine.py
+++ b/gct_plus_amd/engine.py
@@ -16,6 +16,7 @@
 COMPACT_KV = os.environ.get("GCT_COMPACT_KV", "1") != "0"
 COMPACT_FWD = os.environ.get("GCT_COMPACT_FWD", "1") != "0"
 COMPACT_ENC_KV = os.environ.get("GCT_COMPACT_ENC_KV", "1") != "0"
+FOLD_PASSES = os.environ.get("GCT_FOLD_PASSES", "1") != "0"
 
 
 GRAD_NOTIFY = None
@@ -289,7 +290,7 @@
         q, k, v, ldq, ldkv = qb, kvb, kvb[:, d:], d, 2 * d
     site_p = run.site()
     o, lse, probs = ops.attn_fwd(q, k, v, ldq, ldkv, ldkv, mask_u8, B, H, Lq, Lk, dk, run.p,
-                                 run.seed, site_p, want_probs=want_probs, keys=keys, live=live)
+                                 run.seed, site_p, want_probs=want_probs, keys=keys, live=live, zero_gaps=FOLD_PASSES)
     y = _empty(Mq, d, xq)
     site_o = run.site()
     if resid is not None:
@@ -310,9 +311,10 @@
     Mq, Mk = B * Lq, sv.xkv.shape[0]
     kt = run.kt
     new = lambda cols: _empty(Mq, cols, dy)
+    fold = FOLD_PASSES and ops.attn_bwd_zeroes_gaps(Lk)
     if live is not None:
         Mq, kt = live.Mc, None
-        new = live.empty_zero_gaps
+        new = live.empty if fold else live.empty_zero_gaps
         o_in, xq_in = (sv.o, sv.xq) if live.fwd else (live.gather(sv.o), live.gather(sv.xq))
     else:
         o_in, xq_in = sv.o, sv.xq
@@ -329,7 +331,7 @@
         ops.attn_bwd(sv.qb, sv.qb[:, d:], sv.qb[:, 2 * d:], 3 * d, 3 * d, 3 * d, sv.mask_u8, sv.o, do, sv.lse, dqkv,
                      dqkv[:, d:], dqkv[:, 2 * d:], 3 * d, 3 * d, 3 * d, B, H, Lq, Lk, dk, run.p,
                      run.seed, sv.site_p, live=live, kv_compact=live is not None and not fwdc,
-                     keys=live if fwdc else None)
+                     keys=live if fwdc else None, zero_gaps=fold and live is not None)
         segs = [dqkv, dqkv[:, d:], dqkv[:, 2 * d:]]
         ops.linear_wgrad(segs, 3 * d, xq_in,
                          [G(m.q_linear.weight), G(m.k_linear.weight), G(m.v_linear.weight)],
@@ -342,15 +344,18 @@
         if keys is None:
             dkv = _empty(Mk, 2 * d, dy)
         else:
-            dkv = keys.empty_zero_gaps(2 * d)
+            dkv = keys.empty(2 * d) if fold else keys.empty_zero_gaps(2 * d)
         ops.attn_bwd(sv.qb, sv.kvb, sv.kvb[:, d:], d, 2 * d, 2 * d, sv.mask_u8, sv.o, do, sv.lse, dq, dkv, dkv[:, d:],
-                     d, 2 * d, 2 * d, B, H, Lq, Lk, dk, run.p, run.seed, sv.site_p, live=live, keys=keys)
+                     d, 2 * d, 2 * d, B, H, Lq, Lk, dk, run.p, run.seed, sv.site_p, live=live, keys=keys,
+                     zero_gaps=fold and (live is not None or keys is not None))
         ops.linear_wgrad([dq], d, xq_in, [G(m.q_linear.weight)], [G(m.q_linear.bias)], kt=kt)
         ops.linear_wgrad([dkv, dkv[:, d:]], 2 * d, sv.xkv,
                          [G(m.k_linear.weight), G(m.v_linear.weight)],
                          [G(m.k_linear.bias), G(m.v_linear.bias)])
         ops.linear_dgrad([dq], d, Mq, [m.q_linear.weight], dxq_out, depi=depi_q)
-        if sv.self_split:
+        if sv.self_split and FOLD_PASSES:
+            ops.linear_dgrad([dkv, dkv[:, d:]], 2 * d, Mk, [m.k_linear.weight, m.v_linear.weight], dxq_out, scatter=keys)
+        elif sv.self_split:
             dxk = keys.empty(d)
             ops.linear_dgrad([dkv, dkv[:, d:]], 2 * d, Mk, [m.k_linear.weight, m.v_linear.weight], dxk)
             keys.scatter_add(dxk, dxq_out)
@@ -493,11 +498,12 @@
 def encoder_trunk_bwd(enc, run: Run, sv: EncoderSaved, dy, G: GradSink):
     layers, B, L = sv.layers, sv.B, sv.L
     d, nc = enc.d_model, enc.nconds
-    g = dy.reshape(B * L, d).clone()
+    dy = _f32c(dy).reshape(B * L, d)
+    g = torch.empty_like(dy) if FOLD_PASSES else dy.clone()
     gdbuf = torch.empty_like(g) if (run.p > 0 and len(layers) > 0) else None
     dr = _ffn_drop(run, layers[-1].ffn if layers else None, gdbuf)
-    ops.norm_bwd(g, sv.x_last, enc.norm.alpha, sv.mean, sv.rstd, G(enc.norm.alpha), G(enc.norm.bias), out=g,
-                 eps=enc.norm.eps, drop=dr)
+    ops.norm_bwd(dy if FOLD_PASSES else g, sv.x_last, enc.norm.alpha, sv.mean, sv.rstd, G(enc.norm.alpha),
+                 G(enc.norm.bias), out=g, eps=enc.norm.eps, drop=dr)
     gd = None if dr is None else gdbuf
     for i in range(len(layers) - 1, -1, -1):
         g, gd = enc_layer_bwd(run, enc.layers[i], layers[i], g, G, gd=gd, gdbuf=gdbuf,
@@ -571,17 +577,22 @@
         if COMPACT_BWD and len(dec.layers) > 0 and not torch.cuda.is_current_stream_capturing():
             live = lr if RowPlan.usable_live(lr.host(), B * T) else None
     if live_fwd is not None:
-        g = dy.reshape(live.Mc, d).clone()
+        g0 = _f32c(dy).reshape(live.Mc, d)
     elif live is not None:
-        g = live.gather(dy.reshape(B * T, d))
+        g0 = live.gather(dy.reshape(B * T, d))
     else:
-        g = dy.reshape(B * T, d).clone()
+        g0 = _f32c(dy).reshape(B * T, d)
         run.kt = lr.kt if (lr is not None and (B * T) % 32 == 0) else None
+    if live is not None and live_fwd is None:
+        g = g0
+    else:
+        g = torch.empty_like(g0) if FOLD_PASSES else g0.clone()
+        g0 = g0 if FOLD_PASSES else g
     gdbuf = None
     if run.p > 0 and len(layers) > 0:
         gdbuf = torch.empty_like(g) if live is None else live.empty(d)
     dr = _ffn_drop(run, layers[-1].ffn if layers else None, gdbuf)
-    ops.norm_bwd(g, sv.x_last, dec.norm.alpha, sv.mean, sv.rstd, G(dec.norm.alpha), G(dec.norm.bias), out=g,
+    ops.norm_bwd(g0, sv.x_last, dec.norm.alpha, sv.mean, sv.rstd, G(dec.norm.alpha), G(dec.norm.bias), out=g,
                  eps=dec.norm.eps, live=live, drop=dr)
     gd = None if dr is None else gdbuf
     de = new_de()
diff --git a/gct_plus_amd/ops.py b/gct_plus_amd/ops.py
--- a/gct_plus_amd/ops.py
+++ b/gct_plus_amd/ops.py
@@ -13,7 +13,7 @@
 from ._lib import check
 
 EPI_BIAS, EPI_GELU_DROP, EPI_DROP_RESID, EPI_GELU_DROP_SAVE = 0, 1, 2, 3
-DEPI_STORE, DEPI_ACCUM, DEPI_GELU_BWD, DEPI_MUL_SAVED = 0, 1, 2, 3
+DEPI_STORE, DEPI_ACCUM, DEPI_GELU_BWD, DEPI_MUL_SAVED, DEPI_ACCUM_MAPPED = 0, 1, 2, 3, 4
 
 
 def _L():
@@ -325,8 +325,12 @@
 
 
 def linear_dgrad(dys: Sequence[torch.Tensor], lddy: int, M: int, ws_: Sequence[torch.Tensor], dx,
-                 depi=DEPI_STORE, pre=None, p=0.0, seed=0, site=0, live=None, pre_full=False):
+                 depi=DEPI_STORE, pre=None, p=0.0, seed=0, site=0, live=None, pre_full=False, scatter=None):
     nper, K = ws_[0].shape
+    full_rows = pre.shape[0] if (live is not None and pre is not None and pre_full) else 0
+    if scatter is not None:
+        assert live is None and pre is None and depi == DEPI_STORE and M == scatter.Mc and dx.shape[0] == scatter.M
+        depi, live, full_rows = DEPI_ACCUM_MAPPED, scatter, scatter.M
     d = _seg3(dys)
     w = _seg3(ws_)
     _wait_pending(dx)
@@ -338,8 +342,7 @@
                                     ws_[0].stride(0), wp, pstride, K, _p(dx), dx.stride(0), depi,
                                     _p(pre), p, seed, site, _p(wsb), 0 if wsb is None else wsb.numel() * 4,
                                     None if live is None else _p(live.quad_list),
-                                    pre.shape[0] if (live is not None and pre is not None and pre_full) else 0,
-                                    _st()), "gct_linear_dgrad")
+                                    full_rows, _st()), "gct_linear_dgrad")
 
 
 def nonzero_row_tiles(x2d: torch.Tensor):
@@ -601,25 +604,30 @@
 
 
 def attn_fwd(q, k, v, ld_q, ld_k, ld_v, mask, B, H, Lq, Lk, dk, p, seed, site, out=None,
-             want_probs=False, keys=None, live=None):
+             want_probs=False, keys=None, live=None, zero_gaps=True):
     dev = q.device
+    q_rows = live.Mc if (live is not None and zero_gaps) else 0
     if out is not None:
         o = out
     elif live is not None:
-        o = live.empty_zero_gaps(H * dk)
+        o = live.empty(H * dk) if q_rows else live.empty_zero_gaps(H * dk)
     else:
         o = torch.empty(B * Lq, H * dk, dtype=torch.float32, device=dev)
     lse = torch.empty(B * H * Lq, dtype=torch.float32, device=dev)
     probs = torch.empty(B, H, Lq, Lk, dtype=torch.float32, device=dev) if want_probs else None
     mp, sb, sq, mask_owner = _mb(mask, B, Lq, Lk)
-    check(_L().gct_attn_fwd(_p(q), ld_q, _p(k), ld_k, _p(v), ld_v, mp, sb, sq, _p(o),
-                            o.stride(0), _p(lse), _p(probs), B, H, Lq, Lk, dk,
-                            1.0 / math.sqrt(dk), p, seed, site, None if keys is None else _p(keys.cstart),
-                            None if keys is None else _p(keys.n_b), *_tb(mask_owner),
-                            None if live is None else _p(live.cstart), None if live is None else _p(live.n_b),
-                            _st()), "gct_attn_fwd")
+    check(_L().gct_attn_fwd_gaps(_p(q), ld_q, _p(k), ld_k, _p(v), ld_v, mp, sb, sq, _p(o),
+                                 o.stride(0), _p(lse), _p(probs), B, H, Lq, Lk, dk,
+                                 1.0 / math.sqrt(dk), p, seed, site, None if keys is None else _p(keys.cstart),
+                                 None if keys is None else _p(keys.n_b), *_tb(mask_owner),
+                                 None if live is None else _p(live.cstart), None if live is None else _p(live.n_b),
+                                 q_rows, _st()), "gct_attn_fwd")
     del mask_owner
     return o, lse, probs
+
+
+def attn_bwd_zeroes_gaps(Lk):
+    return Lk <= ATTN_DIRECT_MAX_KEYS
 
 
 _ATTN_BWD_WS = {}
@@ -637,18 +645,22 @@
 
 
 def attn_bwd(q, k, v, ld_q, ld_k, ld_v, mask, o, dout, lse, dq, dk_, dv, ld_dq, ld_dk, ld_dv,
-             B, H, Lq, Lk, dk, p, seed, site, live=None, kv_compact=False, keys=None):
+             B, H, Lq, Lk, dk, p, seed, site, live=None, kv_compact=False, keys=None, zero_gaps=False):
+    if zero_gaps and not attn_bwd_zeroes_gaps(Lk):
+        raise _lib.GctError(f"attn_bwd: only the direct kernels (Lk <= {ATTN_DIRECT_MAX_KEYS}) zero gap rows, Lk = {Lk}")
+    q_rows = live.Mc if (zero_gaps and live is not None) else 0
+    kv_rows = 0 if not zero_gaps else (keys.Mc if keys is not None else (live.Mc if kv_compact else 0))
     ws = _attn_bwd_ws(q.device, int(_L().gct_attn_bwd_ws_bytes(B, H, Lq, Lk)))
     mp, sb, sq, mask_owner = _mb(mask, B, Lq, Lk)
-    check(_L().gct_attn_bwd(_p(q), ld_q, _p(k), ld_k, _p(v), ld_v, mp, sb, sq, _p(o),
-                            _p(dout), o.stride(0), _p(lse), _p(dq), ld_dq, _p(dk_), ld_dk,
-                            _p(dv), ld_dv, B, H, Lq, Lk, dk, 1.0 / math.sqrt(dk), p, seed, site,
-                            None if live is None else _p(live.cstart), None if live is None else _p(live.n_b),
-                            int(bool(kv_compact)) | (2 if (live is not None and live.fwd) else 0),
-                            None if keys is None else _p(keys.cstart),
-                            None if keys is None else _p(keys.n_b), *_tb(mask_owner), _p(ws),
-                            0 if ws is None else ws.numel(),
-                            _st()), "gct_attn_bwd")
+    check(_L().gct_attn_bwd_gaps(_p(q), ld_q, _p(k), ld_k, _p(v), ld_v, mp, sb, sq, _p(o),
+                                 _p(dout), o.stride(0), _p(lse), _p(dq), ld_dq, _p(dk_), ld_dk,
+                                 _p(dv), ld_dv, B, H, Lq, Lk, dk, 1.0 / math.sqrt(dk), p, seed, site,
+                                 None if live is None else _p(live.cstart), None if live is None else _p(live.n_b),
+                                 int(bool(kv_compact)) | (2 if (live is not None and live.fwd) else 0),
+                                 None if keys is None else _p(keys.cstart),
+                                 None if keys is None else _p(keys.n_b), *_tb(mask_owner), _p(ws),
+                                 0 if ws is None else ws.numel(), q_rows, kv_rows,
+                                 _st()), "gct_attn_bwd")
     del mask_owner
 
 
diff --git a/include/gctplus_hip.h b/include/gctplus_hip.h
--- a/include/gctplus_hip.h
+++ b/include/gctplus_hip.h
@@ -11,7 +11,7 @@
 #define GCT_ERR_ARG (-1)
 #define GCT_ERR_HIP (-2)
 
-#define GCT_ABI_VERSION 20
+#define GCT_ABI_VERSION 21
 
 int gct_version(void);
 const char* gct_last_error(void);
@@ -51,6 +51,7 @@
 #define GCT_DEPI_ACCUM 1
 #define GCT_DEPI_GELU_BWD 2
 #define GCT_DEPI_MUL_SAVED 3
+#define GCT_DEPI_ACCUM_MAPPED 4
 int gct_linear_dgrad(const float* dy0, const float* dy1, const float* dy2, int64_t lddy,
                      int64_t M, int nseg, int nper,
                      const float* w0, const float* w1, const float* w2, int64_t ldw,
@@ -119,6 +120,20 @@
                  const int32_t* kstart, const int32_t* klen, const uint32_t* tbits, int64_t tb_sb, int64_t tb_su,
                  void* ws, int64_t ws_bytes, void* stream);
 int64_t gct_attn_bwd_ws_bytes(int B, int H, int Lq, int Lk);
+int gct_attn_fwd_gaps(const float* q, int64_t ldq, const float* k, int64_t ldk, const float* v,
+                      int64_t ldv, const uint32_t* mbits, int64_t mb_sb, int64_t mb_sq,
+                      float* o, int64_t ldo, float* lse, float* probs, int B, int H, int Lq, int Lk,
+                      int dk, float scale, float p, uint64_t seed, uint32_t site, const int32_t* kstart,
+                      const int32_t* klen, const uint32_t* tbits, int64_t tb_sb, int64_t tb_su,
+                      const int32_t* qstart, const int32_t* qlen, int64_t q_rows, void* stream);
+int gct_attn_bwd_gaps(const float* q, int64_t ldq, const float* k, int64_t ldk, const float* v,
+                      int64_t ldv, const uint32_t* mbits, int64_t mb_sb, int64_t mb_sq,
+                      const float* o, const float* dout, int64_t ldo, const float* lse,
+                      float* dq, int64_t lddq, float* dk_, int64_t lddk, float* dv, int64_t lddv,
+                      int B, int H, int Lq, int Lk, int dk, float scale, float p, uint64_t seed,
+                      uint32_t site, const int32_t* cstart, const int32_t* nlive, int kv_compact,
+                      const int32_t* kstart, const int32_t* klen, const uint32_t* tbits, int64_t tb_sb, int64_t tb_su,
+                      void* ws, int64_t ws_bytes, int64_t q_rows, int64_t kv_rows, void* stream);
 
 int gct_reparam_fwd(const float* mu, const float* log_var, const float* eps_in, float* eps_out,
                     float* z, int64_t n, uint64_t seed, uint32_t site, void* stream);
```

Result: no change. 11090 (-0.2%).
